# drtconway/zotmer

Measured on AMD Instinct MI355X. Metric: Gk-mers/sec kmerize k=25 on synthetic 150bp FASTQ; achieved HBM GB/s fraction, higher is better.
Workload: dtype u64

## Files before the change

### include/zotk.h

```cpp
#ifndef ZOTK_H
#define ZOTK_H

#include <stdint.h>

#ifdef __cplusplus
extern "C" {
#endif

#define ZK_OK 0
#define ZK_EINVAL (-1)
#define ZK_ENOMEM (-2)
#define ZK_EHIP (-3)
#define ZK_ENOSPC (-4)
#define ZK_EOVERFLOW (-5)
#define ZK_EINTERNAL (-6)
#define ZK_ERANGE (-7)

typedef struct zk_ctx zk_ctx;

zk_ctx* zk_create(int device, uint64_t workspace_bytes);
void zk_destroy(zk_ctx* ctx);
const char* zk_last_error(zk_ctx* ctx);
int zk_set_stream(zk_ctx* ctx, void* hip_stream);
void* zk_get_stream(zk_ctx* ctx);
int zk_sync(zk_ctx* ctx);
int zk_reserve(zk_ctx* ctx, uint64_t workspace_bytes);
int zk_release_workspace(zk_ctx* ctx);
int zk_mem_info(zk_ctx* ctx, uint64_t* free_bytes, uint64_t* total_bytes);
int zk_alloc(zk_ctx* ctx, uint64_t bytes, void** d_ptr);
int zk_free(zk_ctx* ctx, void* d_ptr);
int zk_upload(zk_ctx* ctx, void* d_dst, const void* src, uint64_t bytes);
int zk_download(zk_ctx* ctx, void* dst, const void* d_src, uint64_t bytes);
int zk_copy(zk_ctx* ctx, void* d_dst, const void* d_src, uint64_t bytes);
int zk_host_alloc(zk_ctx* ctx, uint64_t bytes, void** ptr);
int zk_host_free(zk_ctx* ctx, void* ptr);
int zk_upload_async(zk_ctx* ctx, void* d_dst, const void* src, uint64_t bytes);

#define ZK_TUNE_SORT_VARIANT 1
#define ZK_TUNE_PAIRS_VARIANT 2
#define ZK_TUNE_SHORT_SORT 3
#define ZK_TUNE_XCD_GROUP 5
#define ZK_TUNE_SIDE_DIV 4
#define ZK_TUNE_EARLY_COLLAPSE 7
#define ZK_TUNE_PACKED_PAIRS 8
#define ZK_TUNE_WIDE_TILES 9
#define ZK_TUNE_STREAM_PASS 10
#define ZK_TUNE_STREAM_RANGES 11
#define ZK_TUNE_TAG_WORDS 12
#define ZK_TUNE_DEDUPE_VARIANT 13
#define ZK_TUNE_DEDUPE_LIMIT 14
#define ZK_TUNE_DEDUPE_BITS 15
#define ZK_TUNE_COMM_CHUNK 6
#define ZK_TUNE_TAG_PASS 17
#define ZK_TUNE_KWAY 18
#define ZK_TUNE_TILE_SORT 19
#define ZK_TUNE_STRAND_BLOCKS 20
#define ZK_TUNE_COMM_SELF_LOOP 16
int zk_tune(zk_ctx* ctx, int what, int value);

#define ZK_PROF_HIST_STREAM 1
#define ZK_PROF_HIST_ARRAY 2
#define ZK_PROF_PASS_STREAM 3
#define ZK_PROF_PASS_KEYS 4
#define ZK_PROF_PASS_PAIRS 5
#define ZK_PROF_RLE 6
#define ZK_PROF_UNION 7
#define ZK_PROF_SELECT 8
#define ZK_PROF_MIRROR 9
#define ZK_PROF_INTERSECT 10
#define ZK_PROF_COUNT_HIST 11
#define ZK_PROF_PASS_PACKED 12
#define ZK_PROF_SAMPLE 13
#define ZK_PROF_TILE_SORT 14
#define ZK_PROF_CAPTURE_HITS 15
#define ZK_PROF_PROJECT_SUM 16
#define ZK_PROF_SPECTRUM 17
#define ZK_PROF_STRAND_KEYS 18
#define ZK_PROF_STRAND_PAIRS 19
#define ZK_PROF_FORMAT_PAIRS 20
#define ZK_PROF_PROBE_SCAN 21
#define ZK_PROF_BAIT_TALLY 22
#define ZK_PROF_VARS_SCAN 23
#define ZK_PROF_LINKS 24
#define ZK_PROF_LINKS_RC 25
#define ZK_PROF_CONTIG_RENDER 26
#define ZK_PROF_PILEUP 27
#define ZK_PROF_PILEUP_CUT 28
#define ZK_PROF_PULLDOWN_TALLY 29
#define ZK_PROF_CAPTURE_KMERS 30
#define ZK_PROF_PATH_SCAN 31
#define ZK_PROF_LCP_RESOLVE 32
#define ZK_PROF_SCAN_PLACE 33
#define ZK_PROF_SEQ_TALLY 34
#define ZK_PROF_SPIKE_PAIRS 35
#define ZK_PROF_SPIKE_SIZE 36
#define ZK_PROF_KSNP_FLANK 37
#define ZK_PROF_KSNP_PAIRS 38
int zk_debug_buffer(zk_ctx* ctx, void* d_buf);
int zk_profile(zk_ctx* ctx, int enable);
int zk_profile_read(zk_ctx* ctx, int tag, uint64_t* launches, double* total_ms, uint64_t* algorithmic_bytes);


int zk_pack_reads(zk_ctx* ctx, const uint8_t* d_bases, const uint64_t* d_offs, uint64_t n_reads, uint8_t* d_stream);

int zk_encode(zk_ctx* ctx, const uint8_t* d_stream, uint64_t n_bytes, int K, int both,
              uint64_t* d_out, uint64_t cap, uint64_t* n_out, uint64_t acgt[4]);

int zk_subsample(zk_ctx* ctx, const uint64_t* d_kmers, uint64_t n, uint64_t seed, double p,
                 uint64_t* d_out, uint64_t cap, uint64_t* n_out);
// ... 203 lines not shown


int zk_trim(zk_ctx* ctx, const uint64_t* d_kmers, const void* d_counts, int count_bits, uint64_t n,
            uint64_t lo, uint64_t hi, uint64_t* d_ok, void* d_oc, uint64_t cap, uint64_t* n_out);


int zk_codec64_encode(const uint64_t* vals, uint64_t n, int delta, uint64_t* words, uint64_t cap, uint64_t* n_words);
int zk_codec64_count(const uint64_t* words, uint64_t nw, uint64_t* n_values);
int zk_codec64_decode(const uint64_t* words, uint64_t nw, int delta, uint64_t* out, uint64_t cap, uint64_t* n_out);

int zk_codec64_encode_dev(zk_ctx* ctx, const uint64_t* d_vals, uint64_t n, int delta, uint64_t* d_words, uint64_t cap, uint64_t* n_words);
int zk_codec64_decode_dev(zk_ctx* ctx, const uint64_t* d_words, uint64_t nw, int delta, uint64_t* d_out, uint64_t cap, uint64_t* n_out);
int zk_codec64_encode_u32_dev(zk_ctx* ctx, const uint32_t* d_vals, uint64_t n, uint64_t* d_words, uint64_t cap, uint64_t* n_words);

int zk_undelta(zk_ctx* ctx, uint64_t* d_vals, uint64_t n, uint64_t base);
int zk_add_u64(zk_ctx* ctx, uint64_t* d_vals, uint64_t n, uint64_t x);

int zk_parse_fastq(const char* buf, uint64_t len, int final, uint64_t state[4], uint8_t* out, uint64_t out_cap,
                   uint64_t* out_len, uint64_t* consumed);
int zk_parse_fasta(const char* buf, uint64_t len, int final, uint64_t state[4], uint8_t* out, uint64_t out_cap,
                   uint64_t* out_len, uint64_t* consumed);

int zk_fastq_mask(zk_ctx* ctx, const uint8_t* d_text, uint64_t n, uint32_t line_phase, uint8_t* d_stream, uint64_t* n_newlines);

typedef struct zk_source zk_source;
zk_source* zk_source_open(zk_ctx* ctx, const char* path, int threads);
int zk_source_is_gzip(zk_source* src);
int zk_source_start(zk_source* src, uint8_t* d_dst, uint64_t cap);
int zk_source_finish(zk_source* src, uint64_t* n_bytes, int* eof);
void zk_source_close(zk_source* src);
int zk_last_newline(zk_ctx* ctx, const uint8_t* d_text, uint64_t n, uint64_t* cut);
int zk_device_to_file(zk_ctx* ctx, const void* d_src, uint64_t bytes, int fd, uint64_t file_offset, int threads);
int zk_file_to_device(zk_ctx* ctx, int fd, uint64_t file_offset, uint64_t bytes, void* d_dst, int threads);


int zk_synth_reads(zk_ctx* ctx, uint64_t seed, uint64_t first, uint64_t count, int L, uint64_t genome,
                   uint32_t sub_thr, uint32_t n_thr, uint8_t* d_stream);

int zk_checksum(zk_ctx* ctx, const uint64_t* d_kmers, const uint32_t* d_counts, uint64_t n, uint64_t sums[3]);

int zk_first_descent(zk_ctx* ctx, const uint64_t* d_kmers, uint64_t n, uint64_t* first_bad);

int zk_checksum_counts(zk_ctx* ctx, const uint64_t* d_kmers, const void* d_counts, int count_bits, uint64_t n, uint64_t sums[3]);

int zk_synth_keys(zk_ctx* ctx, uint64_t seed, uint64_t first, uint64_t count, int key_bits, uint64_t mul, uint64_t add, uint64_t mod,
                  uint64_t* d_out);
int zk_synth_counts(zk_ctx* ctx, uint64_t seed, const uint64_t* d_keys, uint64_t n, uint64_t* d_counts);

int zk_stream_checksum(zk_ctx* ctx, const uint8_t* d_stream, uint64_t n_bytes, int K, uint64_t sums[7]);

#define ZK_KEYS_FORWARD 0
#define ZK_KEYS_BOTH 1
#define ZK_KEYS_CANONICAL 2

#ifdef __cplusplus
}
#endif
#endif
```

### zotmer_amd/csrc/context.hip

```cpp
#include <stdarg.h>
#include <string.h>

#include "internal.hpp"
#include <vector>

namespace zk {

int fail(zk_ctx* c, int code, const char* fmt, ...) {
    char buf[512];
    va_list ap;
    va_start(ap, fmt);
    vsnprintf(buf, sizeof buf, fmt, ap);
    va_end(ap);
    if (c) c->last_error = buf;
    return code;
}

void arena_reset(zk_ctx* c) { c->arena_off = 0; }

int arena_alloc(zk_ctx* c, uint64_t bytes, void** p) {
    const uint64_t need = (bytes + 255) & ~255ull;
    if (c->arena_off + need > c->arena_size) {
        if (c->arena_off != 0)
            return fail(c, ZK_ENOMEM, "workspace too small: %llu bytes in use, %llu more needed, %llu reserved (call zk_reserve)",
// ... 250 lines not shown
    enter(c);
    if (workspace_bytes <= c->arena_size) return ZK_OK;
    arena_reset(c);
    void* p;
    ZK_TRY(arena_alloc(c, workspace_bytes, &p));
    arena_reset(c);
    return ZK_OK;
}

int zk_release_workspace(zk_ctx* c) {
    if (!c) return ZK_EINVAL;
    enter(c);
    ZK_HIP(c, hipStreamSynchronize(c->stream));
    if (c->arena) { ZK_HIP(c, hipFree(c->arena)); c->arena = nullptr; c->arena_size = 0; c->arena_off = 0; }
    if (c->aux) { ZK_HIP(c, hipFree(c->aux)); c->aux = nullptr; c->aux_size = 0; }
    if (c->status) { ZK_HIP(c, hipFree(c->status)); c->status = nullptr; c->status_words = 0; c->epoch = 0; }
    if (c->part16) { ZK_HIP(c, hipFree(c->part16)); c->part16 = nullptr; c->part16_words = 0; }
    return ZK_OK;
}

int zk_mem_info(zk_ctx* c, uint64_t* free_bytes, uint64_t* total_bytes) {
    if (!c) return ZK_EINVAL;
    enter(c);
    size_t f = 0, t = 0;
    ZK_HIP(c, hipMemGetInfo(&f, &t));
    if (free_bytes) *free_bytes = f;
    if (total_bytes) *total_bytes = t;
    return ZK_OK;
}

int zk_tune(zk_ctx* c, int what, int value) {
    if (!c) return ZK_EINVAL;
    enter(c);
    if (what == ZK_TUNE_SORT_VARIANT) { c->sort_variant = value; return ZK_OK; }
    if (what == ZK_TUNE_PAIRS_VARIANT) { c->pairs_variant = value; return ZK_OK; }
    if (what == ZK_TUNE_SHORT_SORT) { c->short_sort = value; return ZK_OK; }
    if (what == ZK_TUNE_SIDE_DIV) { c->side_div = value; return ZK_OK; }
    if (what == ZK_TUNE_WIDE_TILES) { c->wide_tiles = value ? 1 : 0; return ZK_OK; }
    if (what == ZK_TUNE_PACKED_PAIRS) { c->packed_pairs = value ? 1 : 0; return ZK_OK; }
    if (what == ZK_TUNE_EARLY_COLLAPSE) { c->early_collapse = value < 0 ? 0 : (value > 3 ? 3 : value); return ZK_OK; }
    if (what == ZK_TUNE_COMM_SELF_LOOP) { c->comm_self_loop = value ? 1 : 0; return ZK_OK; }
    if (what == ZK_TUNE_COMM_CHUNK) { c->comm_chunk_bytes = value > 0 ? (uint64_t)value : 0; return ZK_OK; }
    if (what == ZK_TUNE_STREAM_PASS) {
#ifdef ZK_PHASES
        c->stream_pass = value < 0 ? 0 : value;
#else
        if (value < 0 || value > 3) return fail(c, ZK_EINVAL, "stream pass variant %d (0, 1, 2 or 3)", value);
        c->stream_pass = value;
#endif
        return ZK_OK;
    }
    if (what == ZK_TUNE_TAG_WORDS) { c->tag_words = value < 0 ? 0 : (value > 2 ? 2 : value); return ZK_OK; }
    if (what == ZK_TUNE_DEDUPE_VARIANT) { c->dedupe_variant = value < 0 ? -1 : (value & 3); return ZK_OK; }
    if (what == ZK_TUNE_KWAY) { c->kway = value < 0 ? 0 : (value > 2 ? 2 : value); return ZK_OK; }
    if (what == ZK_TUNE_TILE_SORT) { c->tile_sort = value ? 1 : 0; return ZK_OK; }
    if (what == ZK_TUNE_TAG_PASS) { c->tag_pass = value ? 1 : 0; return ZK_OK; }
    if (what == ZK_TUNE_DEDUPE_BITS) { c->dedupe_bits = value < 0 ? 0 : value; return ZK_OK; }
    if (what == ZK_TUNE_STRAND_BLOCKS) { c->strand_blocks = value < 0 ? 0 : (value > 5 ? 1 : value); return ZK_OK; }
    if (what == ZK_TUNE_DEDUPE_LIMIT) { c->dedupe_limit = value < 1 ? 1 : (value > 65536 ? 65536 : value); return ZK_OK; }
    if (what == ZK_TUNE_STREAM_RANGES) { c->stream_ranges = value < 0 ? 0 : (value > 4096 ? 4096 : value); return ZK_OK; }
    if (what == ZK_TUNE_XCD_GROUP) {
        if (value < 0 || value > 32 || (value & (value - 1))) return fail(c, ZK_EINVAL, "xcd group must be 0 or a power of two <= 32");
        c->xcd_group = value;
        return ZK_OK;
    }
    return fail(c, ZK_EINVAL, "unknown tuning knob %d", what);
}

int zk_debug_buffer(zk_ctx* c, void* d_buf) {
    if (!c) return ZK_EINVAL;
    enter(c);
    c->dbg = (u64*)d_buf;
    return ZK_OK;
}

int zk_profile(zk_ctx* c, int enable) {
    if (!c) return ZK_EINVAL;
    enter(c);
    ZK_HIP(c, hipStreamSynchronize(c->stream));
    for (auto& r : c->prof) { (void)hipEventDestroy(r.a); (void)hipEventDestroy(r.b); }
    c->prof.clear();
    c->profile = enable != 0;
    return ZK_OK;
}

int zk_profile_read(zk_ctx* c, int tag, uint64_t* launches, double* total_ms, uint64_t* total_bytes) {
    if (!c) return ZK_EINVAL;
    enter(c);
    ZK_HIP(c, hipStreamSynchronize(c->stream));
    uint64_t n = 0, bytes = 0;
    double ms = 0;
    for (auto& r : c->prof) {
        if (r.tag != tag) continue;
        float t = 0;
        ZK_HIP(c, hipEventElapsedTime(&t, r.a, r.b));
        n++; ms += t; bytes += r.bytes;
    }
    if (launches) *launches = n;
    if (total_ms) *total_ms = ms;
    if (total_bytes) *total_bytes = bytes;
    return ZK_OK;
}

int zk_alloc(zk_ctx* c, uint64_t bytes, void** dptr) {
    if (!c || !dptr) return ZK_EINVAL;
    enter(c);
// ... 66 lines not shown
```

### zotmer_amd/csrc/dedupe.hpp

```cpp
#pragma once
#include "internal.hpp"

namespace zk {

struct DedupeArgs {
    const u64* kin;
    const u32* tin;
    u64 n;
    const u64* cuts;
    u64* out;
    u64* nwords;
    int tag_bits;
    int pack;
    u32* flags;
    u32* counter;
    u64* big;
    u32* n_big;
    u32 big_cap;
    u32 chunks;
    u32* sub;
    u32* bad;
    u32* n_bad;
    u32 bad_cap;
    const u32* list;
    u32* retry;
    u32* n_retry;
    u32 limit;
    u64* dbg;
    u64* m_out;
    u64* m_cursor;
    u64 m_cap;
    u64* m_hist;
    int m_K, m_passes, m_shift[2], m_bits[2];
};

#ifdef ZK_PHASES
#define DD_PHASE(k) do { if (a.dbg) { const u32 now__ = (u32)__builtin_amdgcn_s_memtime(); ph[k] += now__ - tlast; tlast = now__; } } while (0)
#else
#define DD_PHASE(k) do { } while (0)
#endif

int launch_dedupe2(zk_ctx* c, const DedupeArgs& a, bool tagin, int variant, bool unsorted);

}
```

### zotmer_amd/csrc/dedupe2.hip

```cpp
#include "dedupe.hpp"
#include <type_traits>

namespace zk {

template <int BLOCK_, int BATCH_, int ITEMS_>
struct Dedupe2Smem {
    static constexpr int BLOCK = BLOCK_, BATCH = BATCH_, ITEMS = ITEMS_, TILE = BLOCK * ITEMS, NW = BLOCK / 64, ALL = 11264, SPT = ALL / BLOCK,
                         NB = 1024, SIDE = 64 + 64 * BATCH;
    static_assert(ALL % BLOCK == 0 && ALL % 8 == 0 && ITEMS % BATCH == 0 && ITEMS % 4 == 0, "whole rounds, whole quads, whole batches");
    alignas(16) u32 keys[ALL];
    alignas(16) u32 cnt[ALL / 2];
    union {
        u32 side[NW][SIDE];
        struct { u32 bc[NB]; u32 bbase[NB + 1]; } g;
    };
    u32 ticket;
    u32 nout;
};
template <int BLOCK_, int BATCH_, int ITEMS_>
struct Dedupe2MirrorSmem : Dedupe2Smem<BLOCK_, BATCH_, ITEMS_> {
    u32 bins[2][MIRROR_RADIX];
    u64 mbase;
};

template <int ITEMS>
struct Dedupe2Next {
    u32 chunk;
    u64 lo;
    u32 len;
    u32 tag[ITEMS];
};

template <int BLOCK, int ITEMS, bool TAGIN>
__device__ __forceinline__ void dedupe2_load(const DedupeArgs& a, u64 lo, u32 pos, u32 rem, u32 tmask, u32 (&t)[ITEMS]) {
    constexpr u32 TILE = BLOCK * ITEMS;
    u32 tid = threadIdx.x;
    asm volatile("" : "+v"(tid));
    if constexpr (TAGIN) {
        const u32* tp = a.tin + lo + pos;
        if (rem >= TILE) {
            struct __attribute__((packed, aligned(4))) Tag4 { u32 a, b, c, d; };
            static_assert(ITEMS % 4 == 0, "whole quads");
#pragma unroll
            for (int i = 0; i < ITEMS / 4; i++) {
                const Tag4 q = *reinterpret_cast<const Tag4*>(tp + (u32)i * (4 * BLOCK) + 4 * tid);
                t[4 * i] = q.a; t[4 * i + 1] = q.b; t[4 * i + 2] = q.c; t[4 * i + 3] = q.d;
            }
        } else {
#pragma unroll
            for (int i = 0; i < ITEMS; i++) {
                const u32 g = (u32)i * BLOCK + tid;
                t[i] = g < rem ? tp[g] : 0u;
            }
        }
    } else {
        const u64* kp = a.kin + lo + pos;
#pragma unroll
        for (int i = 0; i < ITEMS; i++) {
            const u32 g = (u32)i * BLOCK + tid;
            t[i] = g < rem ? (u32)kp[g] & tmask : 0u;
        }
    }
}

template <class S, bool TAGIN, bool UNSORTED, bool MIRROR>
__device__ __forceinline__ void dedupe2_block(const DedupeArgs& a, S& sm, Dedupe2Next<S::ITEMS>& st, u32 (&ph)[8], u32& tlast) {
    constexpr int BLOCK = S::BLOCK, BATCH = S::BATCH, ITEMS = S::ITEMS, TILE = S::TILE, ALL = S::ALL, SPT = S::SPT, NB = S::NB;
    static_assert(!MIRROR || UNSORTED, "the mirror words are written beside the unsorted ones");
    constexpr u32 EMPTY = ~0u;
    constexpr u32 HS = ALL - 1;
    int tid = threadIdx.x;
    asm volatile("" : "+v"(tid));
    const int lane = tid & 63, wave = __builtin_amdgcn_readfirstlane(tid >> 6);
// ... 201 lines not shown
    __syncthreads();
    DD_PHASE(4);
    next_block(nchunk);
    const u64 hi_part = (u64)chunk << a.tag_bits;
    constexpr int E = 3;
    for (u32 i0 = (u32)tid; i0 < total; i0 += E * BLOCK) {
        u32 mine[E], cc[E], g0[E], g1[E], rank[E];
#pragma unroll
        for (int e = 0; e < E; e++) {
            const u32 i = i0 + e * BLOCK;
            mine[e] = sm.keys[i < total ? i : 0u];
            cc[e] = cnt16[i < total ? i : 0u];
        }
#pragma unroll
        for (int e = 0; e < E; e++) {
            const u32 b = (mine[e] >> bsh) & (NB - 1);
            g0[e] = sm.g.bbase[b]; g1[e] = sm.g.bbase[b + 1];
        }
        u32 o[E][4];
#pragma unroll
        for (int e = 0; e < E; e++)
#pragma unroll
            for (int r = 0; r < 4; r++) o[e][r] = sm.keys[g0[e] + r < (u32)ALL ? g0[e] + r : (u32)ALL - 1];
#pragma unroll
        for (int e = 0; e < E; e++) {
            rank[e] = 0;
#pragma unroll
            for (int r = 0; r < 4; r++) rank[e] += (g0[e] + r < g1[e] && o[e][r] < mine[e]) ? 1u : 0u;
            for (u32 q = g0[e] + 4; q < g1[e]; q += 4) {
                u32 p4[4];
#pragma unroll
                for (int r = 0; r < 4; r++) p4[r] = sm.keys[q + r < (u32)ALL ? q + r : (u32)ALL - 1];
#pragma unroll
                for (int r = 0; r < 4; r++) rank[e] += (q + r < g1[e] && p4[r] < mine[e]) ? 1u : 0u;
            }
        }
#pragma unroll
        for (int e = 0; e < E; e++) {
            const u32 i = i0 + e * BLOCK;
            if (i >= total) break;
            const u32 c = cc[e];
            const u64 k = hi_part | (u64)mine[e];
            if (c > maxc) {
                const u32 at = atomicAdd(a.n_big, 1u);
                if (at < a.big_cap) { a.big[2 * (u64)at] = k; a.big[2 * (u64)at + 1] = c; }
                atomicOr(a.flags, 2u);
            }
            a.out[lo + g0[e] + rank[e]] = (k << a.pack) | (u64)(c > maxc ? 0u : c);
        }
    }
    DD_PHASE(5);
}

template <int BLOCK, int BATCH, int ITEMS, bool TAGIN, bool UNSORTED, bool MIRROR = false>
__global__ __launch_bounds__(BLOCK, 2 * BLOCK / 256) void dedupe2_kernel(DedupeArgs a) {
    using S = typename std::conditional<MIRROR, Dedupe2MirrorSmem<BLOCK, BATCH, ITEMS>, Dedupe2Smem<BLOCK, BATCH, ITEMS>>::type;
    __shared__ S sm;
    static_assert(sizeof(S) <= 80 * 1024, "two workgroups per CU");
    Dedupe2Next<ITEMS> st;
    if constexpr (MIRROR)
        for (int q = threadIdx.x; q < 2 * MIRROR_RADIX; q += BLOCK) (&sm.bins[0][0])[q] = 0;
    if (threadIdx.x == 0) sm.ticket = atomicAdd(a.counter, 1u);
    __syncthreads();
    st.chunk = (u32)__builtin_amdgcn_readfirstlane((int)sm.ticket);
    st.lo = 0; st.len = 0;
    const u32 tmask = a.tag_bits >= 32 ? ~0u : (1u << a.tag_bits) - 1u;
    if (st.chunk < a.chunks) {
        const u64 nlo = a.cuts[st.chunk], nhi = a.cuts[st.chunk + 1];
        st.lo = nlo;
        st.len = nhi - nlo < (u64)a.limit ? (u32)(nhi - nlo) : ~0u;
    }
    if (st.len - 1u < ~0u - 1u) dedupe2_load<BLOCK, ITEMS, TAGIN>(a, st.lo, 0, st.len, tmask, st.tag);
    __syncthreads();
    u32 ph[8] = {0, 0, 0, 0, 0, 0, 0, 0};
    u32 tlast = a.dbg ? (u32)__builtin_amdgcn_s_memtime() : 0u;
    (void)tlast;
    u32 nblk = 0;
    while (st.chunk < a.chunks) {
        dedupe2_block<S, TAGIN, UNSORTED, MIRROR>(a, sm, st, ph, tlast);
        __syncthreads();
        DD_PHASE(6);
        nblk++;
    }
    if constexpr (MIRROR) {
        for (int q = threadIdx.x; q < a.m_passes * MIRROR_RADIX; q += BLOCK) {
            const u32 x = (&sm.bins[0][0])[q];
            if (x) atomicAdd(&a.m_hist[q], (u64)x);
        }
    }
    if (a.dbg && threadIdx.x == 0 && blockIdx.x < 256) {
        for (int k = 0; k < 8; k++) a.dbg[(u64)blockIdx.x * 16 + k] = ph[k];
        a.dbg[(u64)blockIdx.x * 16 + 8] = nblk;
    }
}

int launch_dedupe2(zk_ctx* c, const DedupeArgs& a, bool tagin, int variant, bool unsorted) {
    const u32 want = 2u * (u32)c->num_cus;
    const u32 grid = a.chunks < want ? a.chunks : want;
    if (a.m_out) {
        if (!tagin || !unsorted || !a.m_cursor || !a.m_hist || a.m_passes < 1 || a.m_passes > 2 || a.m_bits[0] > MIRROR_RBITS || a.m_bits[1] > MIRROR_RBITS)
            return fail(c, ZK_EINTERNAL, "launch_dedupe2: mirror words with %d passes, tags %d, unsorted %d", a.m_passes, (int)tagin, (int)unsorted);
        if ((variant & 3) == 1) hipLaunchKernelGGL((dedupe2_kernel<512, 1, 8, true, true, true>), dim3(grid), dim3(512), 0, c->stream, a);
        else hipLaunchKernelGGL((dedupe2_kernel<512, 2, 8, true, true, true>), dim3(grid), dim3(512), 0, c->stream, a);
        ZK_HIP(c, hipGetLastError());
        return ZK_OK;
    }
#define ZK_DD2(N, T, U) hipLaunchKernelGGL((dedupe2_kernel<512, N, 8, T, U>), dim3(grid), dim3(512), 0, c->stream, a)
#define ZK_DD2B(T, U) switch (variant & 3) { case 1: ZK_DD2(1, T, U); break; case 2: ZK_DD2(2, T, U); break; default: ZK_DD2(4, T, U); break; }
    if (unsorted) {
        if (tagin) ZK_DD2B(true, true) else ZK_DD2B(false, true)
    } else {
        if (tagin) ZK_DD2B(true, false) else ZK_DD2B(false, false)
    }
#undef ZK_DD2B
#undef ZK_DD2
    ZK_HIP(c, hipGetLastError());
    return ZK_OK;
}

}
```

### zotmer_amd/csrc/dedupe_blocks.hip

```cpp
#include "internal.hpp"
#include "dedupe.hpp"

namespace zk {

template <bool TAG32>
struct DedupeSmem {
    static constexpr int BLOCK = 1024, ITEMS = 8, TILE = BLOCK * ITEMS, NW = BLOCK / 64, ALL = TAG32 ? 12288 : 6144, SPT = ALL / BLOCK, NB = 256;
    static constexpr int SIDE_KEEP = 128, SIDE = SIDE_KEEP + 64 * ITEMS;
    typedef typename std::conditional<TAG32, u32, u64>::type E;
    E keys[ALL];
    u32 cnt[ALL];
    E side[NW][SIDE];
    u32 bc[NB];
    u32 bbase[NB + 1];
    u32 bfill[NB];
    u32 ticket;
};

__global__ void dedupe_cuts_kernel(const u64* __restrict__ k, u64 n, int tag_bits, u32 blocks, u64* __restrict__ cuts) {
    const u32 v = blockIdx.x * blockDim.x + threadIdx.x;
    if (v > blocks) return;
    u64 lo = 0, hi = n;
    while (lo < hi) {
        const u64 mid = (lo + hi) >> 1;
// ... 332 lines not shown

static int dedupe_lists(zk_ctx* c, const u64* keys, uint64_t n, int key_bits, int b, int pack, u64* work, uint64_t max_chunks,
                        const u32* tags, const u64* tag_cuts, bool unsorted, bool two_per_cu, const DedupeMirror* mirror, DedupeArgs& a, DedupeResult* r) {
    uint64_t chunks = 1ull << b;
    if (max_chunks && chunks > max_chunks) chunks = max_chunks;
    u64 *cuts, *nwords, *incl, *big;
    if (tags) {
        if (!tag_cuts || key_bits - b > 32) return fail(c, ZK_EINTERNAL, "dedupe_pass: tags of %d bits", key_bits - b);
        cuts = const_cast<u64*>(tag_cuts);
    } else ZK_TRY(arena_alloc(c, sizeof(u64) * (chunks + 1), (void**)&cuts));
    ZK_TRY(arena_alloc(c, sizeof(u64) * chunks, (void**)&nwords));
    ZK_TRY(arena_alloc(c, sizeof(u64) * chunks, (void**)&incl));
    ZK_TRY(arena_alloc(c, sizeof(u64) * 2 * DEDUPE_BIG_CAP, (void**)&big));
    a.tag_bits = key_bits - b;
    if (!tags) hipLaunchKernelGGL(dedupe_cuts_kernel, dim3((u32)div_up(chunks + 1, 256)), dim3(256), 0, c->stream, keys, (u64)n, a.tag_bits, (u32)chunks, cuts);
    a.kin = keys; a.tin = tags; a.n = n; a.cuts = cuts; a.out = work; a.nwords = nwords; a.pack = pack;
    a.chunks = (u32)chunks;
    a.flags = (u32*)&c->d_scalars->dedupe_flags;
    a.counter = (u32*)&c->d_scalars->dedupe_counter;
    a.n_big = (u32*)&c->d_scalars->dedupe_n_big;
    a.big = big; a.big_cap = DEDUPE_BIG_CAP;
    ZK_TRY(arena_alloc(c, sizeof(u32) * DEDUPE_BAD_CAP, (void**)&a.bad));
    a.bad_cap = DEDUPE_BAD_CAP;
    a.n_bad = (u32*)&c->d_scalars->dedupe_n_bad;
    a.dbg = c->dbg ? c->dbg + 8192 : nullptr;
    unsorted = unsorted && two_per_cu;
    if (!max_chunks && !unsorted && a.tag_bits >= 14 && c->arena_size - c->arena_off > 64ull * chunks * (4 + 8 + 8) + (32ull << 20) + n / 16)
        ZK_TRY(arena_alloc(c, sizeof(u32) * 64 * chunks, (void**)&a.sub));
    if (mirror && mirror->out && mirror->cap && unsorted && tags && !max_chunks && c->sort_variant == 3) {
        const PassPlan plan = sort_plan_upper(c, key_bits + pack, key_bits + pack - b);
        if (plan.passes <= 2) {
            ZK_TRY(arena_alloc(c, sizeof(u64) * MAX_PASSES * MIRROR_RADIX, (void**)&a.m_hist));
            ZK_HIP(c, hipMemsetAsync(a.m_hist, 0, sizeof(u64) * MAX_PASSES * MIRROR_RADIX, c->stream));
            a.m_out = mirror->out; a.m_cap = mirror->cap; a.m_K = mirror->K; a.m_passes = plan.passes;
            a.m_cursor = &c->d_scalars->dedupe_m_cursor;
            r->mh.passes = plan.passes; r->mh.raw = a.m_hist;
            for (int p = 0; p < plan.passes; p++) { a.m_shift[p] = r->mh.shift[p] = plan.shift[p]; a.m_bits[p] = r->mh.bits[p] = plan.bits[p]; }
            r->m_words = a.m_out; r->m_cap = a.m_cap;
        }
    }
    ZK_HIP(c, hipMemsetAsync(&c->d_scalars->dedupe_flags, 0, ZK_SPAN(dedupe_flags, dedupe_m_cursor), c->stream));
    r->cuts = cuts; r->nwords = nwords; r->incl = incl; r->big = big; r->chunks = (uint32_t)chunks; r->pack = pack; r->work = work;
    r->tag_bits = a.tag_bits; r->unsorted = unsorted;
    return ZK_OK;
}

static void launch_one_per_cu(zk_ctx* c, const DedupeArgs& d) {
    const u32 grid = d.chunks < (u32)c->num_cus ? d.chunks : (u32)c->num_cus;
    if (d.tin) hipLaunchKernelGGL((dedupe_kernel<true, true>), dim3(grid), dim3(1024), 0, c->stream, d);
    else if (d.tag_bits <= 32) hipLaunchKernelGGL((dedupe_kernel<true, false>), dim3(grid), dim3(1024), 0, c->stream, d);
    else hipLaunchKernelGGL((dedupe_kernel<false, false>), dim3(grid), dim3(1024), 0, c->stream, d);
}

static int dedupe_launch(zk_ctx* c, DedupeArgs& a, bool two_per_cu, bool unsorted, DedupeResult* r) {
    prof_begin(c, ZK_PROF_RLE, (a.tin ? 4 : 8) * a.n);
    if (two_per_cu) {
        ZK_TRY(arena_alloc(c, sizeof(u32) * a.chunks, (void**)&a.retry));
        a.n_retry = (u32*)&c->d_scalars->dedupe_n_retry;
        a.limit = (u32)c->dedupe_limit;
        ZK_TRY(launch_dedupe2(c, a, a.tin != nullptr, c->dedupe_variant, unsorted));
    } else launch_one_per_cu(c, a);
    prof_end(c);
    ZK_HIP(c, hipGetLastError());
    ZK_TRY(fetch_span(c, &c->h_scalars->dedupe_flags, ZK_SPAN(dedupe_flags, dedupe_m_cursor)));
    ZK_TRY(fetch(c, &c->h_scalars->dedupe_n_in, a.cuts + a.chunks));
    ZK_TRY(check_device_error(c));
    if (two_per_cu) { r->retry = a.retry; r->n_retry = (uint32_t)c->h_scalars->dedupe_n_retry; }
    if (a.m_out) {
        r->m_placed = c->h_scalars->dedupe_m_cursor;
        r->m_emitted = !((uint32_t)c->h_scalars->dedupe_flags & 4u) && r->m_placed <= a.m_cap;
    }
    if (two_per_cu && (uint32_t)c->h_scalars->dedupe_n_retry) {
        DedupeArgs d = a;
        d.list = a.retry; d.chunks = (uint32_t)c->h_scalars->dedupe_n_retry; d.retry = nullptr; d.n_retry = nullptr;
        ZK_HIP(c, hipMemsetAsync(a.counter, 0, sizeof(u32), c->stream));
        launch_one_per_cu(c, d);
        ZK_HIP(c, hipGetLastError());
        ZK_TRY(fetch_span(c, &c->h_scalars->dedupe_flags, ZK_SPAN(dedupe_flags, dedupe_m_cursor)));
        ZK_TRY(check_device_error(c));
    }
    return ZK_OK;
}

static int dedupe_bad_blocks(zk_ctx* c, const DedupeArgs& a, uint32_t n_bad, DedupeResult* r) {
    uint32_t list[DEDUPE_BAD_CAP];
    ZK_HIP(c, hipMemcpy(list, a.bad, sizeof(u32) * n_bad, hipMemcpyDeviceToHost));
    for (uint32_t i = 0; i < n_bad && !(r->flags & 1); i++) {
        u64 lohi[2];
        ZK_HIP(c, hipMemcpy(lohi, a.cuts + list[i], 2 * sizeof(u64), hipMemcpyDeviceToHost));
        const uint64_t m = lohi[1] - lohi[0];
        u64* res = nullptr;
        u64* bk = const_cast<u64*>(a.kin) + lohi[0];
        if (a.tin) {
            ZK_TRY(arena_alloc(c, 8 * m, (void**)&bk));
            ZK_TRY(expand_tags(c, a.tin, a.cuts, a.chunks, a.tag_bits, bk - lohi[0], list[i], 1));
        }
        ZK_TRY(sort_keys(c, bk, a.out + lohi[0], m, a.tag_bits, &res));
        if (res != bk) ZK_HIP(c, hipMemcpyAsync(bk, res, 8 * m, hipMemcpyDeviceToDevice, c->stream));
        uint64_t u = 0;
        bool ovf = false;
        ZK_TRY(rle(c, bk, m, a.out + lohi[0], nullptr, m, &u, a.pack, &ovf));
        if (ovf) { r->flags |= 1; break; }
        ZK_HIP(c, hipMemcpy(a.nwords + list[i], &u, sizeof(u64), hipMemcpyHostToDevice));
    }
    return ZK_OK;
}

int dedupe_pass(zk_ctx* c, const u64* keys, uint64_t n, int key_bits, int b, int pack, u64* work, uint64_t cap, DedupeResult* r,
                uint64_t* n_in, uint64_t max_chunks, const u32* tags, const u64* tag_cuts, bool unsorted, const DedupeMirror* mirror) {
    *r = DedupeResult();
    if (n_in) *n_in = n;
    if (n == 0) return ZK_OK;
    if (b < 1 || b > 24 || b >= key_bits || pack < 10 || pack > 31) return fail(c, ZK_EINTERNAL, "dedupe_pass: %d block bits of %d, pack %d", b, key_bits, pack);
    if (cap < n) return fail(c, ZK_ENOSPC, "dedupe_pass: work buffer of %llu words for %llu keys", (unsigned long long)cap, (unsigned long long)n);
    DedupeArgs a = {};
    const bool two_per_cu = key_bits - b <= 32 && c->dedupe_variant >= 0;
    ZK_TRY(dedupe_lists(c, keys, n, key_bits, b, pack, work, max_chunks, tags, tag_cuts, unsorted, two_per_cu, mirror, a, r));
    ZK_TRY(dedupe_launch(c, a, two_per_cu, r->unsorted, r));
    r->flags = (uint32_t)c->h_scalars->dedupe_flags;
    r->n_big = (uint32_t)c->h_scalars->dedupe_n_big;
    if (r->n_big > DEDUPE_BIG_CAP) r->flags |= 1;
    const uint32_t n_bad = (uint32_t)c->h_scalars->dedupe_n_bad;
    if (n_bad && n_bad <= DEDUPE_BAD_CAP && !(r->flags & 1) && !max_chunks) {
        ZK_TRY(dedupe_bad_blocks(c, a, n_bad, r));
        a.sub = nullptr;
    } else if (n_bad > DEDUPE_BAD_CAP) r->flags |= 1;
    ZK_HIP(c, hipMemcpyAsync(r->incl, r->nwords, sizeof(u64) * r->chunks, hipMemcpyDeviceToDevice, c->stream));
    ZK_TRY(scan64_inclusive(c, r->incl, r->chunks));
    ZK_TRY(fetch(c, &c->h_scalars->dedupe_n_out, r->incl + r->chunks - 1));
    ZK_TRY(stream_sync(c));
    r->n_out = c->h_scalars->dedupe_n_out;
    prof_add_bytes(c, ZK_PROF_RLE, 8 * r->n_out);
    r->sub = a.sub;
    if (n_in) *n_in = c->h_scalars->dedupe_n_in;
    return ZK_OK;
}

int dedupe_finish(zk_ctx* c, const DedupeResult& r, u64* out_k, u32* out_c, u64* out_m, int K, int gbases, u64** mirror_hist,
                  int* mirror_group_bits, bool packed_out) {
    if (mirror_hist) *mirror_hist = nullptr;
    int gbits = 2 * gbases;
    if (mirror_group_bits) *mirror_group_bits = gbits;
    if (r.n_out == 0) return ZK_OK;
    u64 *minc = nullptr, *place24 = nullptr;
    if (out_m && (1ull << (2 * gbases)) != r.chunks) return fail(c, ZK_EINTERNAL, "dedupe_finish: %u blocks are not 4^%d", r.chunks, gbases);
    if (out_m && r.sub && mirror_group_bits && 2 * K - gbits - 6 >= 8) {
        const uint64_t runs = 64ull * r.chunks;
        u64* minc24;
        ZK_TRY(arena_alloc(c, sizeof(u64) * runs, (void**)&minc24));
        ZK_TRY(arena_alloc(c, sizeof(u64) * runs, (void**)&place24));
        hipLaunchKernelGGL(dedupe_mirror_sizes24_kernel, dim3((u32)div_up(runs, 256)), dim3(256), 0, c->stream, r.sub, r.chunks, gbases, minc24);
        ZK_TRY(scan64_inclusive(c, minc24, runs));
        hipLaunchKernelGGL(dedupe_mirror_place24_kernel, dim3((u32)div_up(runs, 256)), dim3(256), 0, c->stream, r.sub, minc24, r.chunks, gbases, place24);
        ZK_HIP(c, hipGetLastError());
        gbits += 6;
        *mirror_group_bits = gbits;
    }
    MirrorHist mh = {};
    if (out_m && mirror_hist && c->sort_variant == 3) {
        const PassPlan plan = make_plan(2 * K - gbits, MIRROR_RBITS, gbits + r.pack);
        if (plan.passes <= 4) {
            ZK_TRY(arena_alloc(c, sizeof(u64) * MAX_PASSES * MIRROR_RADIX, (void**)&mh.raw));
            ZK_HIP(c, hipMemsetAsync(mh.raw, 0, sizeof(u64) * MAX_PASSES * MIRROR_RADIX, c->stream));
            mh.passes = plan.passes;
            for (int p = 0; p < plan.passes; p++) { mh.shift[p] = plan.shift[p]; mh.bits[p] = plan.bits[p]; }
            *mirror_hist = mh.raw;
        }
    }
    if (out_m && !place24) {
        ZK_TRY(arena_alloc(c, sizeof(u64) * r.chunks, (void**)&minc));
        hipLaunchKernelGGL(dedupe_mirror_sizes_kernel, dim3((r.chunks + 255) / 256), dim3(256), 0, c->stream, r.nwords, r.chunks, gbases, minc);
// ... 14 lines not shown
```

### zotmer_amd/csrc/encode_tile.hpp

```cpp
#pragma once
#include "common.hpp"

namespace zk {

template <int T> struct TileImage {
    static constexpr int NCH = T / 16 + 3;
    u32 codes[NCH];
    u32 valid[NCH];
};

__device__ __forceinline__ u32 record_of_thread(u32 t, u32 cpr, u32 inv) {
    return cpr == 1u ? t : (u32)(((u64)t * inv) >> 32);
}

__device__ __forceinline__ uint4 load_chunk16(const u8* __restrict__ stream, u64 n_bytes, u64 off) {
    uint4 q = make_uint4(0, 0, 0, 0);
    if (off + 16 <= n_bytes) {
        q = *reinterpret_cast<const uint4*>(stream + off);
    } else if (off < n_bytes) {
        u32 w[4] = {0, 0, 0, 0};
        for (int b = 0; b < 16; b++) {
            u32 c = (off + b < n_bytes) ? stream[off + b] : 0u;
            w[b >> 2] |= c << (8 * (b & 3));
        }
        q = make_uint4(w[0], w[1], w[2], w[3]);
    }
    return q;
}

__device__ __forceinline__ void encode_words16(const uint4 q, u32& codes, u32& vmask);

__device__ __forceinline__ void encode_chunk16(const u8* __restrict__ stream, u64 n_bytes, u64 off,
                                               u32& codes, u32& vmask) {
    encode_words16(load_chunk16(stream, n_bytes, off), codes, vmask);
}

__device__ __forceinline__ void encode_words16(const uint4 q, u32& codes, u32& vmask) {
    const u32 w[4] = {q.x, q.y, q.z, q.w};
    u32 cc = 0, vv = 0;
#pragma unroll
    for (int i = 0; i < 4; i++) {
#pragma unroll
        for (int b = 0; b < 4; b++) {
            u32 c = (w[i] >> (8 * b)) & 0xffu;
            u32 t = (c >> 1) & 3u;
            u32 code = t ^ (t >> 1);
            u32 d = (c | 0x20u) - 0x61u;
            u32 ok = (d <= 20u) ? ((0x180045u >> d) & 1u) : 0u;
            cc = (cc << 2) | code;
            vv = (vv << 1) | ok;
        }
    }
    codes = cc;
    vmask = vv;
}

// ... 99 lines not shown
```

### zotmer_amd/csrc/internal.hpp

```cpp
#pragma once
#include <hip/hip_runtime.h>
#include <stddef.h>
#include <stdint.h>
#include <stdio.h>
#include <string>
#include <vector>

#include "../../include/zotk.h"
#include "common.hpp"

struct zk_strand_counters { u32 n_declined, fail; };
struct zk_scalars {
    u64 rle_side;
    u64 total;
    u64 acgt[4];
    u64 n_keys;
    u64 rec_info[3];
    u64 sample_n;
    u64 dedupe_flags, dedupe_n_retry, dedupe_counter, dedupe_n_big, dedupe_n_bad;
    u64 dedupe_m_cursor;
    u64 dedupe_n_in;
    u64 dedupe_n_out;
    zk_strand_counters strand;
    u64 hist_big_n;
// ... 16 lines not shown
    u64 strand_sums[2];
    u64 strand_n_pairs;
    u64 format_bytes;
    u64 compact_total;
    u64 project_heads;
    u64 project_total;
    u64 spectrum[8];
    u64 table_verdict;
    u64 vars[4];
    u64 links_bad;
    u64 render_bad;
    u64 render_bytes;
    u64 pileup_cursor;
    u64 pileup_long;
    u64 pulldown_vetoed;
    u64 capkmers_bad;
    u64 capkmers_total;
    u64 path_total;
    u64 place_bad;
    u64 place_slots;
    u64 seqtally[4];
    u64 spike_bad;
    u64 spike_total[2];
    u64 ksnp_lists[2];
    u64 ksnp_tiles;
};
#define ZK_SPAN(first, last) (offsetof(zk_scalars, last) + sizeof(zk_scalars::last) - offsetof(zk_scalars, first))
static_assert(sizeof(zk_scalars) == 88 * sizeof(u64), "zk_scalars: u64 words only, no padding");
static_assert(ZK_SPAN(rle_side, total) == 2 * sizeof(u64), "rle_prefix reads rle_side and total back as one range");
static_assert(ZK_SPAN(total, acgt) == 5 * sizeof(u64), "the merges read total and acgt back as one range");
static_assert(ZK_SPAN(acgt, n_keys) == 5 * sizeof(u64) && ZK_SPAN(acgt, sample_n) == 9 * sizeof(u64),
              "sort_stream reads acgt, n_keys, rec_info and sample_n back as one range");
static_assert(ZK_SPAN(rec_info, sample_n) == 4 * sizeof(u64), "sort_stream clears rec_info and sample_n as one range");
static_assert(offsetof(zk_scalars, dedupe_n_retry) == offsetof(zk_scalars, dedupe_flags) + 8 &&
              offsetof(zk_scalars, dedupe_counter) == offsetof(zk_scalars, dedupe_flags) + 16 &&
              offsetof(zk_scalars, dedupe_n_big) == offsetof(zk_scalars, dedupe_flags) + 24 &&
              ZK_SPAN(dedupe_flags, dedupe_m_cursor) == 6 * sizeof(u64), "dedupe_pass clears and reads its six words as one range");

struct zk_ctx {
    int device = 0;
    hipStream_t stream = nullptr;
    bool own_stream = false;
    int num_cus = 256;
    int sort_variant = 3;
    int short_sort = 0;
    int packed_pairs = 1;
    int wide_tiles = 1;
    int early_collapse = 1;
    int side_div = 8;
    int pairs_variant = 7;
    int stream_pass = 1;
    int tag_words = 2;
    int dedupe_variant = 0;
    int dedupe_limit = 65536;
    int tag_pass = 0;
    int kway = 1;
    int tile_sort = 1;
    int dedupe_bits = 0;
    int strand_blocks = 1;
    int stream_ranges = 0;

    char* arena = nullptr;
    uint64_t arena_size = 0;
    uint64_t arena_off = 0;

    char* aux = nullptr;
    uint64_t aux_size = 0;

    u64* status = nullptr;
    uint64_t status_words = 0;
    unsigned short* part16 = nullptr;
    uint64_t part16_words = 0;
    u32 epoch = 0;
    u32* d_ticket = nullptr;
    u32* d_xticket = nullptr;
    int num_xcd = 1;
    int xcd_group = 0;
    u32 ticket_base = 0;

    u32* d_err = nullptr;
    zk_scalars* d_scalars = nullptr;
    zk_scalars* h_scalars = nullptr;

    std::string last_error;
    u64* dbg = nullptr;

    void* comm = nullptr;
    int comm_world = 1, comm_rank = 0;
    uint64_t comm_chunk_bytes = 0;
    int comm_self_loop = 0;

    void* ring = nullptr;

    struct ProfRec { int tag; uint64_t bytes; hipEvent_t a, b; };
    bool profile = false;
    std::vector<ProfRec> prof;
};

namespace zk {

int fail(zk_ctx* c, int code, const char* fmt, ...);
static inline void enter(zk_ctx* c) {
    int d = -1;
    if (c && (hipGetDevice(&d) != hipSuccess || d != c->device)) (void)hipSetDevice(c->device);
}
#define ZK_HIP(c, call)                                                                         \
// ... 20 lines not shown
void prof_begin(zk_ctx* c, int tag, uint64_t algorithmic_bytes);
void prof_end(zk_ctx* c);
void prof_add_bytes(zk_ctx* c, int tag, uint64_t bytes);

int fetch_span(zk_ctx* c, void* h_first, size_t bytes, const void* from = nullptr);
template <class T> static inline int fetch(zk_ctx* c, T* h_field, const void* from = nullptr) { return fetch_span(c, h_field, sizeof(T), from); }
int stream_sync(zk_ctx* c);

static inline uint64_t div_up(uint64_t a, uint64_t b) { return (a + b - 1) / b; }
static inline u32 grid_cap(const zk_ctx* c, uint64_t blocks, int per_cu) {
    const uint64_t mx = (uint64_t)c->num_cus * per_cu;
    return (u32)(blocks < mx ? blocks : mx);
}

constexpr int MAX_PASSES = 8;
struct PassPlan {
    int passes;
    int shift[MAX_PASSES];
    int bits[MAX_PASSES];
};
static inline PassPlan make_plan(int key_bits, int rbits, int lo = 0) {
    PassPlan p;
    if (key_bits < 1) key_bits = 1;
    if (key_bits > 64) key_bits = 64;
    p.passes = (key_bits + rbits - 1) / rbits;
    int base = key_bits / p.passes, rem = key_bits % p.passes, s = lo;
    for (int i = 0; i < MAX_PASSES; i++) { p.shift[i] = 0; p.bits[i] = 0; }
    for (int i = 0; i < p.passes; i++) {
        p.bits[i] = base + (i < rem ? 1 : 0);
        p.shift[i] = s;
        s += p.bits[i];
    }
    return p;
}
int sort_keys(zk_ctx* c, u64* keys, u64* alt, uint64_t n, int key_bits, u64** result);
int sort_pairs(zk_ctx* c, u64* keys, u64* alt, u32* vals, u32* valt, uint64_t n, int key_bits, u64** rk, u32** rv);
int sort_keys_upper(zk_ctx* c, u64* keys, u64* alt, uint64_t n, int key_bits, int lo_bit, u64** result, int prof_tag = ZK_PROF_PASS_PACKED);
int sort_pairs_upper(zk_ctx* c, u64* keys, u64* alt, u32* vals, u32* valt, uint64_t n, int key_bits, int lo_bit, u64** rk, u32** rv);
int sort_pairs_mirrored(zk_ctx* c, const u64* src_k, const u32* src_v, u64* keys, u64* alt, u32* vals, u32* valt, uint64_t n, int K,
                        u64** rk, u32** rv, int lo_bit = 0);
int sort_pairs_rbits(zk_ctx* c);
struct StreamSample { int shift; uint64_t value; double max_ratio; uint64_t seen = 0, distinct = 0; bool want_distinct = false; };
struct StreamTags { bool written = false; u64* cuts = nullptr; uint32_t blocks = 0; };
struct StreamSrc { const u8* stream; uint64_t n_bytes; int K; int mode; int lo_bit; int hi_bit = 0; StreamSample* sample = nullptr;
                   StreamTags* tags = nullptr; };
int sort_stream(zk_ctx* c, const StreamSrc& src, u64* buf_a, u64* buf_b, uint64_t cap, uint64_t* n_keys,
                uint64_t acgt[4], u64** result);
int sort_rbits(zk_ctx* c);
PassPlan sort_plan_upper(zk_ctx* c, int key_bits, int lo_bit);
int sort_first_bits(zk_ctx* c, int key_bits, int lo_bit);
constexpr int MIRROR_RBITS = 9, MIRROR_RADIX = 1 << MIRROR_RBITS;
struct MirrorHist { int passes; int shift[4]; int bits[4]; u64* raw; };
int sort_keys_upper_counted(zk_ctx* c, u64* keys, u64* alt, uint64_t n, int key_bits, int lo_bit, u64* counted, u64** result);
struct DedupeMirror { u64* out = nullptr; uint64_t cap = 0; int K = 0; };
struct DedupeResult {
    uint64_t n_out = 0;
    uint32_t flags = 0;
    uint32_t n_big = 0;
    u64 *cuts = nullptr, *nwords = nullptr, *incl = nullptr, *big = nullptr, *work = nullptr;
    u32* sub = nullptr;
    uint32_t chunks = 0;
    int pack = 0;
    int tag_bits = 0;
    bool unsorted = false;
    bool m_emitted = false;
    u64* m_words = nullptr;
    uint64_t m_cap = 0, m_placed = 0;
    MirrorHist mh = {};
    u32* retry = nullptr;
    uint32_t n_retry = 0;
};
int dedupe_pass(zk_ctx* c, const u64* keys, uint64_t n, int key_bits, int b, int pack, u64* work, uint64_t cap, DedupeResult* r,
                uint64_t* n_in = nullptr, uint64_t max_chunks = 0, const u32* tags = nullptr, const u64* tag_cuts = nullptr,
                bool unsorted = false, const DedupeMirror* mirror = nullptr);
int expand_tags(zk_ctx* c, const u32* tags, const u64* cuts, uint32_t blocks, int tag_bits, u64* keys_out, uint64_t first_block = 0, uint64_t n_blocks = 0);
int dedupe_finish(zk_ctx* c, const DedupeResult& r, u64* out_k, u32* out_c, u64* out_m = nullptr, int K = 0, int gbases = 0,
                  u64** mirror_hist = nullptr, int* mirror_group_bits = nullptr, bool packed_out = false);
int dedupe_sort_blocks(zk_ctx* c, DedupeResult& r);
int strand_blocks(zk_ctx* c, const DedupeResult& r, u64* keys_buf, uint64_t buf_words, int K, u64* out_k, u32* out_c, uint64_t cap,
                  uint64_t* n_out);
int collapse_pass(zk_ctx* c, const u64* keys, uint64_t n, int shift, int bits, int pack, u64* out, uint64_t cap, uint64_t* n_out,
                  uint64_t max_tiles = 0);
struct StreamRows { u32* rows = nullptr; u64* offs = nullptr; u32 ranges = 0, radix = 0; u32* gcodes = nullptr; u16* gvalid = nullptr;
                    u32 strands = 1;
                    bool wide = false; };
int stream_hist(zk_ctx* c, const u8* stream, uint64_t n_bytes, int K, int mode, const PassPlan& plan, u64* ghist, u32 gstride,
                u64* d_acgt, u64* d_n, u64* rec_info, u64* sample, u32 sample_cap, int sample_shift, u64 sample_value, u32* sample_n,
                void* image_room, uint64_t image_room_bytes, StreamRows* out);
struct StreamPlanes { u16* dig; int shift, bits; };
int stream_pass0(zk_ctx* c, uint64_t n_bytes, int K, int mode, int shift, int bits, const u64* ghist0, const StreamRows& rows,
                 uint64_t first_nl, bool uniform, u64* kout, uint64_t n, int variant, const StreamPlanes* planes = nullptr);
int stream_pass1(zk_ctx* c, const u32* tags, const u16* dig, uint64_t n, const u64* ghist0, uint32_t radix0, int bits1, u32* tout, u64* cuts);
int tile_sort_top_bits(uint64_t n, int key_bits, int rbits);
int tile_sort(zk_ctx* c, u64* keys, u32* vals, uint64_t n, int key_bits, int top, bool* declined);
int tile_sort_count(zk_ctx* c, const u64* keys, uint64_t n, int key_bits, int top, u64* uniq, u32* counts, uint64_t cap, uint64_t* n_unique,
                    bool* declined);
int trim(zk_ctx* c, const u64* keys, const void* cnts, int cbits, uint64_t n, u64 lo, u64 hi, u64* ok, void* oc,
         uint64_t cap, uint64_t* n_out);
int project_dedupe(zk_ctx* c, const u64* keys, uint64_t n, int shift, u64* out, uint64_t cap, uint64_t* n_out);
int subsample(zk_ctx* c, const u64* keys, uint64_t n, u64 seed, double p, u64* out, uint64_t cap, uint64_t* n_out);
int sample_pairs(zk_ctx* c, const u64* keys, const u64* cnts, uint64_t n, u64 seed, double p, u64* ok, u64* oc, uint64_t cap,
                 uint64_t* n_out);
int subsample_pairs(zk_ctx* c, u64* keys, u32* cnts, uint64_t n, u64 seed, double p, uint64_t* n_out);
int encode_list(zk_ctx* c, const u8* stream, uint64_t n_bytes, int K, int both, u64* out, uint64_t cap, uint64_t* n_out,
                uint64_t acgt[4]);
int capture_filter(zk_ctx* c, const u8* stream, uint64_t n_bytes, int K, const u64* baits, uint64_t n_baits, u8* out,
                   uint64_t* n_reads, uint64_t* n_kept);
// ... 37 lines not shown
```

### zotmer_amd/csrc/pipeline.hip

```cpp
#include <string.h>

#include <vector>

#include "internal.hpp"

namespace zk {

__global__ void mirror_kernel(const u64* __restrict__ c, const u32* __restrict__ n, u64 m, int K, u64* __restrict__ r,
                              u32* __restrict__ v) {
    for (u64 i = (u64)blockIdx.x * blockDim.x + threadIdx.x; i < m; i += (u64)gridDim.x * blockDim.x) {
        r[i] = revcomp(K, c[i]);
        v[i] = n[i];
    }
}

constexpr int MIRROR_GROUP_BITS = 18;
constexpr int MIRROR_GROUP_BASES = MIRROR_GROUP_BITS / 2;

__global__ void mirror_bounds_kernel(const u64* __restrict__ c, u64 n, int K, int gbits, u64* __restrict__ start) {
    const u32 g = blockIdx.x * blockDim.x + threadIdx.x;
    if (g > (1u << gbits)) return;
    const u64 want = (u64)g << (2 * K - gbits);
    u64 lo = 0, hi = n;
    if (g == (1u << gbits)) lo = n;
// ... 192 lines not shown
        ZK_TRY(sort_pairs_mirrored(c, sorted, cnt, rk, rk2, rv, rv2, uc, K, &sk, &sv));
    }
    return union_sum(c, sorted, cnt, uc, sk, sv, uc, out_k, out_c, 32, cap, n_out, nullptr, (K & 1) != 0);
}

int mirror_expand(zk_ctx* c, const u64* ck, const u32* cc, uint64_t n, int K, u64* out_k, u32* out_c, uint64_t cap, uint64_t* n_out) {
    *n_out = 0;
    if (K < 1 || K > 32) return fail(c, ZK_EINVAL, "K must be in 1..32 (got %d)", K);
    if (n == 0) return ZK_OK;
    arena_reset(c);
    const uint64_t a8 = align256(8 * n), a4 = align256(4 * n);
    int pack = 0;
    ZK_TRY(mirror_pack(c, K, cc, n, false, 0, &pack));
    const bool words = mirror_as_words(pack, K, n);
    const uint64_t wbytes = 2 * a8 + (words ? 0 : 2 * a4);
    const uint64_t need = wbytes + (9 << 20) + n / 8 + (words && n >= (1ull << 26) ? (480ull << 20) : 0);
    ZK_TRY(arena_require(c, need, need));
    char* w;
    ZK_TRY(arena_alloc(c, wbytes, (void**)&w));
    ZK_TRY(mirror_union(c, ck, cc, n, K, (u64*)w, (u64*)(w + a8), words ? nullptr : (u32*)(w + 2 * a8), words ? nullptr : (u32*)(w + 2 * a8 + a4), out_k, out_c,
                        cap, n_out, pack));
    return check_device_error(c);
}

enum CountRoute {
    COUNT_TILES,
    COUNT_BLOCKS,
    COUNT_FUSED,
    COUNT_RUNS,
    COUNT_SORTED,
    COUNT_REPLAN
};

constexpr double REPEAT_RATIO = 0.6;
static StreamSample prefix_sample(int K, int bits) { return StreamSample{2 * K - bits, (uint64_t)(0x0D71C8E5u >> (32 - bits)), REPEAT_RATIO}; }

struct KmerizePlan {
    int K;
    bool both, canonical_only;
    int rb;
    int pack;
    int collapse_bit;
    int fused_bit;
    int dedupe_bit;
    bool tags;
    int tile_top;
    int both_top;
    bool replan_pays;
    bool look;
    int look_bits;
    bool blocks_mirror;
    bool blocks_strands;
    bool blocks_unsorted;
    CountRoute low_route() const { return fused_bit ? COUNT_FUSED : collapse_bit ? COUNT_RUNS : COUNT_SORTED; }
};

static KmerizePlan plan_kmerize(const zk_ctx* c, uint64_t n_bytes, int K, bool both, bool canonical_only) {
    KmerizePlan p = {};
    p.K = K; p.both = both; p.canonical_only = canonical_only;
    const int rb = p.rb = sort_rbits(const_cast<zk_ctx*>(c));
    p.pack = c->packed_pairs ? pack_bits_for(K) : 0;
    const int lg = ilog2_ceil(n_bytes);
    if (!both && c->early_collapse) {
        const int b = rb * ((lg + 3 + rb - 1) / rb);
        if (b + rb / 2 < 2 * K) p.collapse_bit = b;
        if (p.collapse_bit >= 2 * rb && (c->early_collapse == 1 || c->early_collapse == 3) && p.pack) p.fused_bit = p.collapse_bit - rb;
    }
    if (p.fused_bit && c->early_collapse == 1) {
        const int passes = lg > 15 ? (lg - 15 + rb - 1) / rb : 1;
        const int b = rb * passes;
        if (b < p.fused_bit + rb && b + rb / 2 < 2 * K && b <= 24 && (n_bytes >> b) >= 2048) p.dedupe_bit = b;
    }
    if (!both && c->early_collapse == 1 && c->dedupe_bits > 0 && p.pack && c->dedupe_bits % rb == 0 && c->dedupe_bits + rb / 2 < 2 * K &&
        c->dedupe_bits <= 24)
        p.dedupe_bit = c->dedupe_bits;
    p.tags = p.dedupe_bit && c->tag_words && 2 * K - p.dedupe_bit <= 32;
    p.tile_top = c->tile_sort ? tile_sort_top_bits(n_bytes, 2 * K, rb) : 0;
    p.both_top = tile_sort_top_bits(2 * n_bytes, 2 * K, rb);
    p.replan_pays = !canonical_only && c->tile_sort && p.both_top;
    p.look_bits = lg - 15 < 2 ? 2 : (lg - 15 > 30 ? 30 : lg - 15);
    p.look = !p.dedupe_bit && !both && c->early_collapse && !pack_bits_for(K) && p.tile_top && p.look_bits < 2 * K;
    p.blocks_mirror = !canonical_only && p.pack && p.dedupe_bit == MIRROR_GROUP_BITS && mirror_groups(K);
    p.blocks_strands = p.blocks_mirror && (K & 1) && c->strand_blocks;
    p.blocks_unsorted = p.blocks_mirror && (K & 1) && (c->strand_blocks == 1 || c->strand_blocks >= 3);
    return p;
}

struct SortBufs {
    u64 *a, *b;
    uint64_t cap_keys;
    u64* other(const void* p) const { return p == a ? b : a; }
};
struct Output { u64* k; u32* c; uint64_t cap; uint64_t* n_out; };

struct Sorted {
    u64* keys = nullptr;
    u64* other = nullptr;
    uint64_t n = 0;
    StreamTags tags;
    bool presampled = false;
    CountRoute route = COUNT_SORTED;
};

static int sort_by_plan(zk_ctx* c, const KmerizePlan& p, const u8* stream, uint64_t n_bytes, const SortBufs& b, bool may_replan,
                        uint64_t acgt[4], Sorted* s) {
    const int K = p.K;
    StreamSrc src{stream, n_bytes, K, p.both ? ZK_KEYS_BOTH : ZK_KEYS_CANONICAL, 0};
    s->route = p.dedupe_bit ? COUNT_BLOCKS : p.low_route();
    bool sorted = false;
    if (p.dedupe_bit) {
        StreamSample smp = prefix_sample(K, p.dedupe_bit - 2);
        src.lo_bit = 2 * K - p.dedupe_bit; src.sample = &smp;
        if (p.tags) src.tags = &s->tags;
        const int rc = sort_stream(c, src, b.a, b.b, b.cap_keys, &s->n, acgt, &s->keys);
        if (rc < 0) return rc;
        src.sample = nullptr; src.tags = nullptr;
        if (rc == 1 && may_replan && p.replan_pays) { s->route = COUNT_REPLAN; return ZK_OK; }
        if (rc == 1) s->route = p.tile_top ? COUNT_TILES : p.low_route();
        else sorted = true;
        s->presampled = smp.seen >= 4096;
    } else if (p.look) {
        StreamSample smp = prefix_sample(K, p.look_bits);
        smp.want_distinct = true;
        src.lo_bit = 2 * K - p.tile_top; src.sample = &smp;
        const int rc = sort_stream(c, src, b.a, b.b, b.cap_keys, &s->n, acgt, &s->keys);
        if (rc < 0) return rc;
        src.sample = nullptr;
        if (rc != 1) { s->route = COUNT_TILES; sorted = true; }
    }
    if (!sorted) {
        if (s->route == COUNT_TILES) { src.lo_bit = 2 * K - p.tile_top; src.hi_bit = 0; }
        else { src.lo_bit = 0; src.hi_bit = p.fused_bit ? p.fused_bit : p.collapse_bit; }
        ZK_TRY(sort_stream(c, src, b.a, b.b, b.cap_keys, &s->n, acgt, &s->keys));
    }
    s->other = b.other(s->keys);
    return ZK_OK;
}

enum ListPlace {
    IN_SORT_BUF,
    IN_AUX,
    IN_OUTPUT,
    EMITTED
};
struct Counted {
    u64* keys = nullptr;
    u32* cnt = nullptr;
    uint64_t uc = 0;
    ListPlace where = IN_SORT_BUF;
    bool have_max = false;
    uint64_t max_count = 0;
    u64 *mwords = nullptr, *malt = nullptr;
    u64* mhist = nullptr;
    int mgroup = MIRROR_GROUP_BITS;
};

static int aux_list(zk_ctx* c, uint64_t m, u64** k, u32** v) {
    char* aux;
    ZK_TRY(aux_require(c, align256(8 * m) + align256(4 * m), &aux));
    *k = (u64*)aux; *v = (u32*)(aux + align256(8 * m));
    return ZK_OK;
}

static int count_sorted(zk_ctx* c, const KmerizePlan& p, const SortBufs& b, u64* keys, uint64_t n, const Output& o, Counted* r) {
    if (p.canonical_only) {
        r->where = IN_OUTPUT;
        return rle(c, keys, n, o.k, o.c, o.cap, &r->uc);
    }
    r->keys = keys; r->cnt = (u32*)b.other(keys); r->where = IN_SORT_BUF;
    return rle(c, keys, n, keys, r->cnt, n, &r->uc);
}

constexpr int ALL_BITS = -1;
static int count_by_passes(zk_ctx* c, const KmerizePlan& p, const SortBufs& b, u64* keys, uint64_t n, int lo_bit, const Output& o, Counted* r) {
    u64* res = nullptr;
    if (lo_bit == ALL_BITS) ZK_TRY(sort_keys(c, keys, b.other(keys), n, 2 * p.K, &res));
    else ZK_TRY(sort_keys_upper(c, keys, b.other(keys), n, 2 * p.K, lo_bit, &res, ZK_PROF_PASS_KEYS));
    return count_sorted(c, p, b, res, n, o, r);
}

static int reduce_words(zk_ctx* c, const KmerizePlan& p, u64* words, u64* alt, uint64_t u1, int lo_bit, Counted* r) {
    u64* res = nullptr;
    ZK_TRY(sort_keys_upper(c, words, alt, u1, 2 * p.K + p.pack, lo_bit + p.pack, &res));
    ZK_TRY(aux_list(c, u1, &r->keys, &r->cnt));
    ZK_TRY(reduce_by_key(c, res, nullptr, u1, r->keys, r->cnt, u1, &r->uc, p.pack, &r->max_count));
    r->where = IN_AUX; r->have_max = true;
    return ZK_OK;
}

static int count_tiles(zk_ctx* c, const KmerizePlan& p, const SortBufs& b, const Sorted& s, const Output& o, Counted* r) {
    bool declined = false;
    if (p.canonical_only) ZK_TRY(tile_sort_count(c, s.keys, s.n, 2 * p.K, p.tile_top, o.k, o.c, o.cap, &r->uc, &declined));
    else ZK_TRY(tile_sort_count(c, s.keys, s.n, 2 * p.K, p.tile_top, s.keys, (u32*)s.other, s.n, &r->uc, &declined));
    if (declined) return count_by_passes(c, p, b, s.keys, s.n, 0, o, r);
    r->keys = s.keys; r->cnt = (u32*)s.other; r->where = p.canonical_only ? IN_OUTPUT : IN_SORT_BUF;
    return ZK_OK;
}

static int count_blocks(zk_ctx* c, const KmerizePlan& p, const SortBufs& b, const Sorted& s, const Output& o, zk_kmerize_stats* st, Counted* r) {
    const int K = p.K, pk = p.pack;
    DedupeResult d;
    uint64_t n_in = 0;
    const uint64_t nblocks = 1ull << p.dedupe_bit, per = s.n / nblocks + 1;
    const u32* tg = s.tags.written ? (const u32*)s.keys : nullptr;
    if (!s.presampled) ZK_TRY(dedupe_pass(c, s.keys, s.n, 2 * K, p.dedupe_bit, pk, s.other, b.cap_keys, &d, &n_in, (1u << 20) / per + 4, tg, s.tags.cuts));
    if (s.presampled || (!(d.flags & 1) && (double)d.n_out <= REPEAT_RATIO * (double)n_in)) {
        DedupeMirror mo;
        const uint64_t tag_words = align256(4 * s.n) / 8;
        if (tg && p.blocks_strands && p.blocks_unsorted && c->strand_blocks != 4 && tag_words < b.cap_keys) {
            mo.out = s.keys + tag_words; mo.cap = b.cap_keys - tag_words; mo.K = K;
            if (c->strand_blocks == 5 && mo.cap > 1024) mo.cap = 1024;
        }
        ZK_TRY(dedupe_pass(c, s.keys, s.n, 2 * K, p.dedupe_bit, pk, s.other, b.cap_keys, &d, nullptr, 0, tg, s.tags.cuts, p.blocks_unsorted, &mo));
        if (!(d.flags & 1)) {
            const uint64_t uc = r->uc = d.n_out;
            const bool want_m = !(d.flags & 2) && p.blocks_mirror;
            if (want_m && p.blocks_strands && 2 * align256(8 * uc) <= 8 * b.cap_keys) {
                st->n_canonical = uc;
                r->where = EMITTED;
                return strand_blocks(c, d, s.keys, b.cap_keys, K, o.k, o.c, o.cap, o.n_out);
            }
            if (d.unsorted) ZK_TRY(dedupe_sort_blocks(c, d));
            ZK_TRY(aux_list(c, uc, &r->keys, &r->cnt));
            ZK_TRY(dedupe_finish(c, d, r->keys, r->cnt, want_m ? s.keys : nullptr, K, MIRROR_GROUP_BASES, &r->mhist, &r->mgroup, want_m));
            if (want_m) { r->mwords = s.keys; r->malt = s.other; }
            r->where = IN_AUX;
            if (!(d.flags & 2)) { r->max_count = (1ull << pk) - 1; r->have_max = true; }
            return ZK_OK;
        }
    }
    u64* keys = s.keys;
    if (tg) {
        ZK_TRY(expand_tags(c, tg, s.tags.cuts, s.tags.blocks, 2 * K - p.dedupe_bit, s.other));
        keys = s.other;
    }
    return count_by_passes(c, p, b, keys, s.n, ALL_BITS, o, r);
}

static int count_fused(zk_ctx* c, const KmerizePlan& p, const SortBufs& b, const Sorted& s, const Output& o, Counted* r) {
    const int pk = p.pack;
    const int cb = sort_first_bits(c, 2 * p.K + pk, p.fused_bit + pk);
    const uint64_t sample_tiles = 64, tile_keys = 8192;
    uint64_t us = 0, u1 = 0;
    ZK_TRY(collapse_pass(c, s.keys, s.n, p.fused_bit, cb, pk, s.other, b.cap_keys, &us, sample_tiles));
    const uint64_t m = s.n < sample_tiles * tile_keys ? s.n : sample_tiles * tile_keys;
    if ((double)us > REPEAT_RATIO * (double)m) return count_by_passes(c, p, b, s.keys, s.n, p.fused_bit, o, r);
    ZK_TRY(collapse_pass(c, s.keys, s.n, p.fused_bit, cb, pk, s.other, b.cap_keys, &u1));
    return reduce_words(c, p, s.other, s.keys, u1, p.fused_bit, r);
}

static int count_runs(zk_ctx* c, const KmerizePlan& p, const SortBufs& b, const Sorted& s, const Output& o, Counted* r) {
    const int K = p.K;
    uint64_t m = 0, heads = 0;
    ZK_TRY(sample_heads(c, s.keys, s.n, &m, &heads));
    if ((double)heads > REPEAT_RATIO * (double)m) return count_by_passes(c, p, b, s.keys, s.n, p.collapse_bit, o, r);
    if (p.pack) {
        uint64_t u1 = 0;
        bool ovf = false;
        const int rc1 = rle(c, s.keys, s.n, s.other, nullptr, b.cap_keys, &u1, p.pack, &ovf);
        if (rc1 != ZK_OK && rc1 != ZK_ENOSPC) return rc1;
// ... 296 lines not shown
```

### zotmer_amd/csrc/radix_sort.hip

```cpp
#include <stdlib.h>
#include "internal.hpp"
#include "encode_tile.hpp"

namespace zk {

constexpr int MAX_RADIX = 1024;

enum { SRC_ARRAY = 0, SRC_STREAM = 1 };

template <int BLOCK_, int ITEMS_, int RBITS_, int ROUNDS_ = 1, int WPE_ = 1, int SEG_ = 32, bool PIPE_ = false>
struct Cfg {
    static constexpr int BLOCK = BLOCK_, ITEMS = ITEMS_, RBITS = RBITS_, ROUNDS = ROUNDS_, WPE = WPE_, SEG = SEG_;
    static constexpr bool PIPE = PIPE_;
    static_assert(SEG == 0 || (BLOCK * ITEMS < 32768 && (SEG & (SEG - 1)) == 0), "16-bit tile counts");
    static constexpr int TILE = BLOCK * ITEMS, RADIX = 1 << RBITS, NW = BLOCK / 64;
    static constexpr int EXCH = TILE / ROUNDS, IPR = ITEMS / ROUNDS;
    static_assert(ITEMS % ROUNDS == 0, "ROUNDS");
    static constexpr int DPT = (RADIX + BLOCK - 1) / BLOCK;
    static_assert(ITEMS % 2 == 0 && 2 * ITEMS < 256, "ITEMS");
    static_assert(64 * ITEMS < 65536, "per-wave ranks are 16-bit");
    static_assert(RADIX <= MAX_RADIX && RBITS * MAX_PASSES >= 64, "RBITS");
};

struct SortArgs {
// ... 39 lines not shown

template <class C, int SRC, bool PAIRS, bool COUNT>
__device__ __forceinline__ u32 load_tile(const SortArgs& a, u32 tile, TileImage<C::TILE>* img, u64 (&key)[C::ITEMS],
                                         u32 (&val)[C::ITEMS], u32& acgt) {
    constexpr int TILE = C::TILE, ITEMS = C::ITEMS, BLOCK = C::BLOCK;
    const int lane = threadIdx.x & 63, wave = __builtin_amdgcn_readfirstlane((int)(threadIdx.x >> 6));
    u32 live = 0;
    if (SRC == SRC_ARRAY) {
        const u64 base = (u64)tile * TILE + (u64)wave * (64 * ITEMS) + lane;
#pragma unroll
        for (int i = 0; i < ITEMS; i++) {
            const u64 idx = base + (u64)i * 64;
            const bool ok = idx < a.n;
            key[i] = ok ? a.kin[idx] : 0ull;
            if (PAIRS) val[i] = ok ? a.vin[idx] : 0u;
            live |= (ok ? 1u : 0u) << i;
        }
        if (a.mirror_K > 0) {
#pragma unroll
            for (int i = 0; i < ITEMS; i++) key[i] = revcomp(a.mirror_K, key[i]);
        }
    } else {
        const bool both = (a.mode == ZK_KEYS_BOTH);
        const int pos_per_tile = both ? TILE / 2 : TILE;
        const u64 t0 = (u64)tile * pos_per_tile;
        for (int c = threadIdx.x; c < pos_per_tile / 16 + 3; c += BLOCK) {
            u32 cc, vv;
            encode_chunk16(a.stream, a.n_bytes, t0 + 16ull * c, cc, vv);
            img->codes[c] = cc;
            img->valid[c] = vv;
        }
        __syncthreads();
        const int K = a.K;
        if (both) {
            constexpr int H = ITEMS / 2;
#pragma unroll
            for (int i = 0; i < H; i++) {
                const int p = wave * (64 * H) + i * 64 + lane;
                u64 x;
                const bool ok = window_at(*img, p, K, x);
                const u64 xb = revcomp(K, x);
                key[i] = x;
                key[i + H] = xb;
                live |= (ok ? 1u : 0u) << i;
                live |= (ok ? 1u : 0u) << (i + H);
                if (COUNT && ok) acgt += (1u << (8 * (u32)(x & 3))) + (1u << (8 * (u32)(xb & 3)));
            }
        } else if (ITEMS == 16) {
            u64 xs[16], xr[16];
            const u32 ok16 = windows16(*img, (int)threadIdx.x, K, xs, xr);
#pragma unroll
            for (int i = 0; i < ITEMS; i++) {
                const u64 x = xs[i & 15], xb = xr[i & 15];
                key[i] = (a.mode == ZK_KEYS_CANONICAL) ? (x < xb ? x : xb) : x;
                if (COUNT && ((ok16 >> i) & 1u)) acgt += (1u << (8 * (u32)(x & 3))) + (1u << (8 * (u32)(xb & 3)));
            }
            live = ok16;
        } else {
#pragma unroll
            for (int i = 0; i < ITEMS; i++) {
                const int p = wave * (64 * ITEMS) + i * 64 + lane;
                u64 x;
                const bool ok = window_at(*img, p, K, x);
                const u64 xb = revcomp(K, x);
                key[i] = (a.mode == ZK_KEYS_CANONICAL) ? (x < xb ? x : xb) : x;
                live |= (ok ? 1u : 0u) << i;
                if (COUNT && ok) acgt += (1u << (8 * (u32)(x & 3))) + (1u << (8 * (u32)(xb & 3)));
            }
        }
    }
    return live;
}

struct HistArgs {
    SortArgs src;
    PassPlan plan;
    u64* ghist;
    u64* acgt;
    u32 tiles;
    u64* rec_info;
    u64* sample;
    u32* sample_n;
    u32 sample_cap;
    int sample_shift;
    u64 sample_value;
};

__global__ void first_newline_kernel(const u8* __restrict__ stream, u64 n_bytes, u64* out) {
    __shared__ u32 best;
    if (threadIdx.x == 0) best = 0xffffffffu;
    __syncthreads();
    const u64 lim = n_bytes < 65536 ? n_bytes : 65536;
    for (u64 i = threadIdx.x; i < lim; i += blockDim.x)
        if (stream[i] == '\n') atomicMin(&best, (u32)i);
    __syncthreads();
    if (threadIdx.x == 0) out[0] = (best == 0xffffffffu) ? ~0ull : (u64)best;
}

template <class C, int SRC> struct NextTile;
template <class C> struct NextTile<C, SRC_ARRAY> {
    u64 key[C::ITEMS];
    u32 val[C::ITEMS];
    u32 live = 0;
    template <bool PAIRS = false>
    __device__ __forceinline__ void issue(const SortArgs& a, u32 t, int tid, int wave, int lane) {
        const u64 base = (u64)t * C::TILE + (u64)wave * (64 * C::ITEMS) + lane;
        if ((u64)(t + 1) * C::TILE <= a.n) {
            const u64* p = a.kin + base;
#pragma unroll
            for (int i = 0; i < C::ITEMS; i++) key[i] = p[i * 64];
            if constexpr (PAIRS) {
                const u32* q = a.vin + base;
#pragma unroll
                for (int i = 0; i < C::ITEMS; i++) val[i] = q[i * 64];
            }
            live = (C::ITEMS >= 32) ? ~0u : ((1u << C::ITEMS) - 1u);
            return;
        }
// ... 31 lines not shown
    NextTile<C, SRC_STREAM> nx;
    nx.q0 = nx.q1 = make_uint4(0, 0, 0, 0);
    if (pre && blockIdx.x < h.tiles) nx.issue(h.src, blockIdx.x, threadIdx.x, 0, 0);
    u32 rec = 0, m = 0, step_m = 0, nl_count = 0, bad_count = 0;
    if (PRE && h.rec_info) {
        const u64 first_nl = h.rec_info[0];
        if (first_nl < 0x7fffffffull) {
            rec = (u32)first_nl + 1u;
            m = (u32)(((u64)blockIdx.x * C::TILE + 16ull * threadIdx.x) % rec);
            step_m = (u32)(((u64)gridDim.x * C::TILE) % rec);
        }
    }
    for (u32 tile = blockIdx.x; tile < h.tiles; tile += gridDim.x) {
        u64 key[C::ITEMS];
        u32 val[C::ITEMS];
        u32 pk = 0;
        u32 live = 0;
        if (pre) {
            if constexpr (PREFETCH) {
                if (rec) {
                    const u32 w4[4] = {nx.q0.x, nx.q0.y, nx.q0.z, nx.q0.w};
                    const int sep = (int)(rec - 1u) - (int)m;
                    const u64 off = (u64)tile * C::TILE + 16ull * threadIdx.x;
                    const bool expect = sep >= 0 && sep < 16 && off + (u64)sep < h.src.n_bytes;
                    bool bad = false;
#pragma unroll
                    for (int q = 0; q < 4; q++) {
                        const u32 x = w4[q] ^ 0x0a0a0a0au;
                        const u32 t = ~(((x & 0x7f7f7f7fu) + 0x7f7f7f7fu) | x | 0x7f7f7f7fu);
                        nl_count += (u32)__popc(t);
                        const u32 want = (expect && (sep >> 2) == q) ? (0x80u << (8 * (sep & 3))) : 0u;
                        bad |= (t != want);
                    }
                    bad_count += bad ? 1u : 0u;
                    m += step_m;
                    if (m >= rec) m -= rec;
                }
                u32 cc, vv;
                encode_words16(nx.q0, cc, vv);
                img.codes[threadIdx.x] = cc; img.valid[threadIdx.x] = vv;
                if (threadIdx.x + C::BLOCK < TileImage<C::TILE>::NCH) {
                    encode_words16(nx.q1, cc, vv);
                    img.codes[threadIdx.x + C::BLOCK] = cc; img.valid[threadIdx.x + C::BLOCK] = vv;
                }
                __syncthreads();
                if (tile + gridDim.x < h.tiles) nx.issue(h.src, tile + gridDim.x, threadIdx.x, 0, 0);
                Windows16<C::TILE> wg;
                wg.init(img, (int)threadIdx.x, h.src.K);
#pragma unroll
                for (int i = 0; i < 16; i++) {
                    u64 x, xb;
                    if (wg.get(i, x, xb)) {
                        pk += (1u << (8 * (u32)(x & 3))) + (1u << (8 * (u32)(xb & 3)));
                        const u64 kk = (h.src.mode == ZK_KEYS_CANONICAL) ? (x < xb ? x : xb) : x;
                        if (h.plan.passes == 2) {
                            atomicAdd(&bins[(u32)(kk >> h.plan.shift[0]) & ((1u << h.plan.bits[0]) - 1u)], 1u);
                            atomicAdd(&bins[C::RADIX + ((u32)(kk >> h.plan.shift[1]) & ((1u << h.plan.bits[1]) - 1u))], 1u);
                        } else {
#pragma unroll
                            for (int p = 0; p < MAX_PASSES; p++) {
                                if (p < h.plan.passes) {
                                    const u32 d = (u32)(kk >> h.plan.shift[p]) & ((1u << h.plan.bits[p]) - 1u);
                                    atomicAdd(&bins[p * C::RADIX + d], 1u);
                                }
                            }
                        }
                        if (h.sample && (kk >> h.sample_shift) == h.sample_value) {
                            const u32 at = atomicAdd(h.sample_n, 1u);
                            if (at < h.sample_cap) h.sample[at] = kk;
                        }
                    }
                }
                live = 0;
            }
        } else {
            if constexpr (!PRE) live = load_tile<C, SRC, false, SRC == SRC_STREAM>(h.src, tile, &img, key, val, pk);
        }
        a0 += pk & 0xffu; a1 += (pk >> 8) & 0xffu; a2 += (pk >> 16) & 0xffu; a3 += pk >> 24;
#pragma unroll
        for (int i = 0; i < C::ITEMS; i++) {
            const bool lv = (live >> i) & 1u;
#pragma unroll
            for (int p = 0; p < MAX_PASSES; p++) {
                if (p < h.plan.passes) {
                    const u32 d = (u32)(key[i] >> h.plan.shift[p]) & ((1u << h.plan.bits[p]) - 1u);
                    bool act = lv;
                    if (SRC == SRC_ARRAY) {
#pragma unroll
                        for (int r = 0; r < 2; r++) {
                            const u64 m = __ballot(act);
                            if (m == 0) break;
                            const int leader = __ffsll((long long)m) - 1;
                            const u32 dl = (u32)__builtin_amdgcn_readlane((int)d, leader);
                            const u64 same = __ballot(act && d == dl);
                            if (__popcll(same) < 8) break;
                            if ((int)(threadIdx.x & 63) == leader) atomicAdd(&bins[p * C::RADIX + dl], (u32)__popcll(same));
                            act = act && d != dl;
                        }
                    }
                    if (act) atomicAdd(&bins[p * C::RADIX + d], 1u);
                }
            }
        }
        if (SRC == SRC_STREAM) __syncthreads();
    }
    __syncthreads();
    for (int i = threadIdx.x; i < h.plan.passes * C::RADIX; i += C::BLOCK) {
// ... 444 lines not shown
        u64 key[ITEMS];
        u32 val[PAIRS ? ITEMS : 1];
        u32 rank2[ITEMS / 2];
        u32 live = 0;
        u32 tC = 0;
        bool vC = false;
        bool atomB = false;
        bool early = false;
        u32 tcB[DPT], dexB[DPT];
        u32 incB = 0, tsumB = 0;
        u64 rowA[DPT];
#pragma unroll
        for (int j = 0; j < DPT; j++) { tcB[j] = 0; dexB[j] = 0; rowA[j] = 0; }

        if (vB) {
            if constexpr (SRC == SRC_ARRAY) {
#pragma unroll
                for (int i = 0; i < ITEMS; i++) key[i] = nx.key[i];
                if constexpr (PAIRS) {
#pragma unroll
                    for (int i = 0; i < ITEMS; i++) val[i] = nx.val[i];
                    if (a.mirror_K > 0) {
#pragma unroll
                        for (int i = 0; i < ITEMS; i++) key[i] = revcomp(a.mirror_K, key[i]);
                    }
                }
                live = nx.live;
            } else {
                __syncthreads();
                const u32 nch = a.rec ? (a.rpt * a.rec) / 16 + 3 : (u32)TileImage<TILE>::NCH;
                u32 cc, vv;
                if ((u32)tid < nch) {
                    encode_words16(nx.q0, cc, vv);
                    sm.img.codes[tid] = cc; sm.img.valid[tid] = vv;
                }
                if ((u32)tid + BLOCK < nch) {
                    encode_words16(nx.q1, cc, vv);
                    sm.img.codes[tid + BLOCK] = cc; sm.img.valid[tid + BLOCK] = vv;
                }
                __syncthreads();
                u64 xs[16], xr[16];
                u32 p0 = 16u * tid_o, lim = 0xffffu;
                if (a.rec) {
                    const u32 r = record_of_thread((u32)tid_o, a.cpr, a.cpr_inv), j = tid_o - r * a.cpr;
                    p0 = r * a.rec + 16u * j;
                    const int left = (int)a.wpr - 16 * (int)j;
                    lim = (r < a.rpt) ? ((left >= 16) ? 0xffffu : ((1u << (left > 0 ? left : 0)) - 1u)) : 0u;
                    if (r >= a.rpt) p0 = 0;
                }
                live = windows16_at(sm.img, (int)p0, a.K, xs, xr) & lim;
#pragma unroll
                for (int i = 0; i < ITEMS; i++) {
                    const u64 x = xs[i & 15], xb = xr[i & 15];
                    key[i] = (a.mode == ZK_KEYS_CANONICAL) ? (x < xb ? x : xb) : x;
                }
                __syncthreads();
            }
            if constexpr (ATOM) atomB = !((a.straddle[tB >> 5] >> (tB & 31u)) & 1u);
            if (ATOM && atomB) {
                if (dirty) {
                    __syncthreads();
                    if (tid < RADIX) cnt32[tid] = 0;
                    __syncthreads();
                    dirty = false;
                }
                PSTAMP(tB, 1);
#pragma unroll
                for (int i = 0; i < ITEMS; i++) {
                    const bool lv = (live >> i) & 1u;
                    const u32 d = (u32)(key[i] >> a.shift) & dmask;
                    const u32 r = lv ? atomicAdd(&cnt32[d], 1u) : 0u;
                    if (i & 1) rank2[i / 2] |= r << 16; else rank2[i / 2] = r;
                }
            } else {
            if constexpr (ATOM) dirty = true;
            {
                u32 z = 0;
                asm volatile("" : "+v"(z));
                for (int q = lane; q < RADIX / 8; q += 64) reinterpret_cast<uint4*>(mycnt)[q] = make_uint4(z, z, z, z);
            }
#ifdef ZK_STAMPS
            asm volatile("s_waitcnt vmcnt(0)" ::: "memory");
#endif
            PSTAMP(tB, 1);
#pragma unroll
            for (int i = 0; i < ITEMS; i++) {
                const bool lv = (live >> i) & 1u;
                const u32 d = (u32)(key[i] >> a.shift) & dmask;
                u32 plo, phi;
                match_digit<C::RBITS>(d, __ballot(lv), plo, phi);
                const u32 below = __builtin_amdgcn_mbcnt_hi(phi, __builtin_amdgcn_mbcnt_lo(plo, 0u));
                const u32 npeer = (u32)__popc(plo) + (u32)__popc(phi);
                const u32 pre = lv ? (u32)mycnt[d] : 0u;
                if (i & 1) rank2[i / 2] |= (pre + below) << 16; else rank2[i / 2] = pre + below;
                if (lv && below == npeer - 1) mycnt[d] = (u16)(pre + npeer);
            }
            }
            PSTAMP(tB, 2);
            if constexpr (SRC == SRC_ARRAY) {
#pragma unroll
                for (int i = 0; i < ITEMS; i++) asm volatile("" : "+v"(key[i]));
            }
            if (tid == 0) {
                u32 t = tile_of(myx, pending, a.nx, a.glog);
                if (t >= tiles) t = steal_tile(a, myx, tiles);
                sm.ticket = t;
            }
// ... 172 lines not shown
    const u32 v = blockIdx.x, Rd = 1u << bits_d, Rin = 1u << bits_in;
    for (u32 d = threadIdx.x; d < Rd; d += blockDim.x) corr[d] = 0;
    __syncthreads();
    const u64 boundary = ghist_in[v];
    const u64 tv = boundary / tile;
    for (u64 i = tv * tile + threadIdx.x; i < boundary; i += blockDim.x) atomicAdd(&corr[(u32)(kin[i] >> shift) & (Rd - 1u)], 1u);
    __syncthreads();
    for (u32 d = threadIdx.x; d < Rd; d += blockDim.x) {
        u64 before;
        if (tv < tiles) before = status[tv * stride + d] & ZK_ST_VALUE_MASK;
        else before = (d + 1 < Rd ? ghist_d[d + 1] : n) - ghist_d[d];
        cuts[(u64)d * Rin + v] = ghist_d[d] + before + corr[d];
    }
    if (v == 0 && threadIdx.x == 0) cuts[(u64)Rd * Rin] = n;
}

int launch_wide_pass(zk_ctx* c, const SortArgs& a);

static int straddle_bitmap(zk_ctx* c, uint64_t n, u32 tile, const u64* starts, u32 buckets, u32 radix, const u32** bitmap) {
    const u32 tiles = (u32)div_up(n, tile);
    u32* bm;
    ZK_TRY(arena_alloc(c, sizeof(u32) * (tiles / 32 + 1), (void**)&bm));
    ZK_HIP(c, hipMemsetAsync(bm, 0, sizeof(u32) * (tiles / 32 + 1), c->stream));
    if (starts) {
        hipLaunchKernelGGL(straddle_kernel, dim3((radix + 255) / 256), dim3(256), 0, c->stream, starts, buckets, tile, bm);
        ZK_HIP(c, hipGetLastError());
    }
    *bitmap = bm;
    return ZK_OK;
}

struct RecInfo { uint64_t first_nl; bool uniform; };
static RecInfo uniform_records(const zk_ctx* c, uint64_t n_bytes) {
    const uint64_t first_nl = c->h_scalars->rec_info[0], nl = c->h_scalars->rec_info[1], bad = c->h_scalars->rec_info[2];
    return {first_nl, first_nl < 0x7fffffffull && n_bytes % (first_nl + 1) == 0 && bad == 0 && nl == n_bytes / (first_nl + 1)};
}

static void publish_tags(StreamTags* t, u64* cuts, uint64_t blocks) { t->cuts = cuts; t->blocks = (uint32_t)blocks; t->written = true; }

constexpr u32 SAMPLE_CAP = 1u << 20;
struct StreamPlan {
    int top;
    PassPlan plan;
    bool sampling;
    bool ranged;
    bool planes;
    bool tags;
    bool straddle;
};
static StreamPlan stream_plan(const zk_ctx* c, const StreamSrc& src, uint64_t cap, int rbits, bool pipe, uint64_t n) {
    StreamPlan s;
    s.top = (src.hi_bit > 0 && src.hi_bit < 2 * src.K) ? src.hi_bit : 2 * src.K;
    s.plan = make_plan(s.top - src.lo_bit, rbits, src.lo_bit);
    s.sampling = src.sample && cap >= 4ull * SAMPLE_CAP && src.mode == ZK_KEYS_CANONICAL;
    s.ranged = c->stream_pass != 0;
    const uint64_t n_pad = ((n + 63) & ~63ull) + 64;
    s.planes = s.ranged && c->tag_pass && src.tags && s.plan.passes == 2 && s.plan.shift[0] == 32 && s.plan.bits[0] == 9 && s.plan.bits[1] == 9 &&
               src.mode == ZK_KEYS_CANONICAL && 2 * src.K > 32 && n >= 4096 && 4 * n_pad + 2 * n + 64 <= 8 * cap;
    s.tags = src.tags && pipe && s.plan.passes == 2 && s.plan.shift[0] <= 32 && src.mode == ZK_KEYS_CANONICAL;
    s.straddle = c->tag_words >= 2 && pipe;
    return s;
}

struct RecordTiles { u32 rec = 0, rpt = 0, cpr = 0, wpr = 0, cpr_inv = 0; };
static bool record_tiles(uint64_t first_nl, int K, int block, int tile, int img_words, RecordTiles* t) {
    const uint64_t rec = first_nl + 1;
    const int64_t W = (int64_t)first_nl - K + 1;
    if (rec < 16 || W < 1) return false;
    const uint32_t cpr = (uint32_t)((W + 15) / 16);
    const uint32_t rpt = (block / cpr) / 16 * 16;
    if (!(rpt >= 16 && (uint64_t)rpt * rec / 16 + 3 <= (uint64_t)img_words && (double)rpt * (double)W > 1.02 * (double)tile * (double)W / (double)rec))
        return false;
    t->rec = (u32)rec; t->rpt = rpt; t->cpr = cpr; t->wpr = (u32)W;
    t->cpr_inv = (u32)(((1ull << 32) + cpr - 1) / cpr);
    return true;
}

template <class C>
struct Sorter {
    static int rbits() { return C::RBITS; }
    static u32 tiles_for(const SortArgs& a, int src) {
        if (src == SRC_ARRAY) return (u32)div_up(a.n, C::TILE);
        if (a.rec) return (u32)div_up(a.n_bytes / a.rec, a.rpt);
        const u64 pos = (a.mode == ZK_KEYS_BOTH) ? C::TILE / 2 : C::TILE;
        return (u32)div_up(a.n_bytes, pos);
    }

    static int begin_pass(zk_ctx* c, SortArgs& a, u32 tiles, u32 tickets, bool pipe, bool stamps = true) {
        const bool seg = !pipe && C::SEG > 0;
        ZK_TRY(lookback_begin(c, seg ? ((uint64_t)tiles / (C::SEG > 0 ? C::SEG : 1) + 2) * C::RADIX : (uint64_t)tiles * C::RADIX, tickets,
                              &a.epoch, &a.ticket_base));
        if (pipe || seg) ZK_TRY(part16_begin(c, (uint64_t)tiles * C::RADIX, &a.part));
        a.status = c->status;
        a.ticket = c->d_ticket;
        a.err = c->d_err;
        a.dbg = stamps ? c->dbg : nullptr;
        a.dbg2 = (stamps && c->dbg) ? c->dbg + 8ull * tiles : nullptr;
        return ZK_OK;
    }
    template <bool PAIRS>
    static int begin_pipe(zk_ctx* c, SortArgs& a, u32 tiles, u32* grid, bool stamps) {
        u32 g = (u32)c->num_cus * (sizeof(PipeSmem<C, PAIRS>) > 80 * 1024 ? 1 : 2);
        if (g > tiles) g = tiles;
        g += C::RADIX / 64;
        ZK_TRY(begin_pass(c, a, tiles, g, true, stamps));
        ZK_HIP(c, hipMemsetAsync(c->d_xticket, 0, 8 * 32 * sizeof(u32), c->stream));
        a.xticket = c->d_xticket;
        a.nx = 1u;
        a.glog = 0;
        *grid = g;
        return ZK_OK;
    }
// ... 412 lines not shown
```

### zotmer_amd/csrc/stream_pass.hip

```cpp
#include "internal.hpp"
#include "encode_tile.hpp"

#include <stdlib.h>
#include <type_traits>

namespace zk {

constexpr int P0_BLOCK = 512, P0_NW = 8, P0_TILE = P0_BLOCK * P0_NW, P0_IMG_WORDS = 320;
constexpr int PW_BLOCK = 1024, PW_NW = 8, PW_TILE = PW_BLOCK * PW_NW, PW_IMG_WORDS = 640;
constexpr int SH_BLOCK = 512, SH_NW = 16, SH_TILE = SH_BLOCK * SH_NW;

struct P0Geom { u32 block, nw, img_words; };
__host__ __device__ constexpr P0Geom p0_geom(bool wide) { return wide ? P0Geom{PW_BLOCK, PW_NW, PW_IMG_WORDS} : P0Geom{P0_BLOCK, P0_NW, P0_IMG_WORDS}; }

struct StreamTiling {
    u32 rec;
    u32 rpt, cpr, wpr;
    u32 cpr_inv;
    u32 tile_bytes;
    u32 ranges;
    u64 range_bytes;
};

__host__ __device__ inline StreamTiling make_tiling(u64 n_bytes, u64 first_nl, int K, u32 ranges, P0Geom g) {
// ... 81 lines not shown
    x = (x | (x << 4)) & 0x0F0F0F0Fu;
    x = (x | (x << 2)) & 0x33333333u;
    x = (x | (x << 1)) & 0x55555555u;
    return x;
}

struct SHistArgs {
    const u8* stream;
    u64 n_bytes;
    int K, mode;
    PassPlan plan;
    u32 binbase[MAX_PASSES];
    u32 nbins;
    u64* ghist;
    u32 gstride;
    u32* rows;
    u64* acgt;
    u64* rec_info;
    u64* sample;
    u32* sample_n;
    u32 sample_cap;
    int sample_shift;
    u64 sample_value;
    u32 revbase;
    u32 ranges, split;
    u32* gcodes;
    u16* gvalid;
    int dbg_atomics;
    P0Geom geom;
};

template <bool HI, bool TWO, int CANON_T = -1>
__global__ __launch_bounds__(SH_BLOCK, 4) void stream_hist_kernel(SHistArgs h) {
    extern __shared__ u32 bins[];
    __shared__ TileImage<SH_TILE> img;
    __shared__ u32 pshift[MAX_PASSES], pmask[MAX_PASSES], pbase[MAX_PASSES];
    const int tid = threadIdx.x;
    for (u32 i = tid; i < h.nbins; i += SH_BLOCK) bins[i] = 0;
    if (tid < MAX_PASSES) {
        pshift[tid] = (u32)h.plan.shift[tid] - (HI ? 32u : 0u);
        pmask[tid] = (1u << h.plan.bits[tid]) - 1u;
        pbase[tid] = h.binbase[tid];
    }
    const u64 first_nl = h.rec_info[0];
    const StreamTiling tl = make_tiling(h.n_bytes, first_nl, h.K, h.ranges, h.geom);
    const u32 w = blockIdx.x / h.split, sp = blockIdx.x % h.split;
    const u64 B = (u64)w * tl.range_bytes;
    const u64 E = (B + tl.range_bytes < h.n_bytes) ? B + tl.range_bytes : h.n_bytes;
    const u32 ntile = B < E ? (u32)((E - B + SH_TILE - 1) / SH_TILE) : 0u;
    const int K = h.K;
    const int np = h.plan.passes;
    const u64 mask = ~0ull >> (64 - 2 * K);
    const u32 mlo = (u32)mask, mhi = (u32)(mask >> 32);
    const bool canon = CANON_T == 1 ? true : h.mode == ZK_KEYS_CANONICAL;
    const bool both = CANON_T != 1 && h.mode == ZK_KEYS_BOTH;
    const u32 sh0 = (u32)h.plan.shift[0] - (HI ? 32u : 0u), sh1 = (u32)h.plan.shift[1] - (HI ? 32u : 0u);
    const u32 dm0 = (1u << h.plan.bits[0]) - 1u, dm1 = (1u << h.plan.bits[1]) - 1u;
    const u32 base1 = h.binbase[1];
    const u32 nb0 = (u32)h.plan.bits[0], nb1 = (u32)h.plan.bits[1];
    const u32 ssh = (u32)h.sample_shift - (HI ? 32u : 0u);
    const typename std::conditional<HI, u32, u64>::type sval = (typename std::conditional<HI, u32, u64>::type)h.sample_value;
    u32 a0 = 0, a1 = 0, a2 = 0, a3 = 0, nl_count = 0, bad_count = 0;
    u32 rec = 0, m = 0, step_m = 0;
    if (first_nl < 0x7fffffffull) {
        rec = (u32)first_nl + 1u;
        m = (u32)((B + (u64)sp * SH_TILE + 16ull * tid) % rec);
        step_m = (u32)(((u64)h.split * SH_TILE) % rec);
    }
    uint4 q0 = make_uint4(0, 0, 0, 0), q1 = q0;
    auto issue = [&](u32 j) {
        const u64 P = B + (u64)j * SH_TILE;
        q0 = load_chunk16(h.stream, h.n_bytes, P + 16ull * tid);
        if (tid < 3) q1 = load_chunk16(h.stream, h.n_bytes, P + 16ull * (tid + SH_BLOCK));
    };
    if (sp < ntile) issue(sp);
    __syncthreads();
    for (u32 j = sp; j < ntile; j += h.split) {
        const u64 off = B + (u64)j * SH_TILE + 16ull * tid;
        const bool mine = off < E;
        {
            u32 cc, vv;
            encode_swar16(q0, cc, vv);
            if (rec) {
                if (mine) {
                    const int sep = (int)(rec - 1u) - (int)m;
                    const bool expect = sep >= 0 && sep < 16 && off + (u64)sep < h.n_bytes;
                    const u32 sepbit = expect ? (0x8000u >> (sep & 15)) : 0u;
                    if ((vv | sepbit) == 0xffffu) {
                        const u32 wsel = (sep & 12) == 0 ? q0.x : (sep & 12) == 4 ? q0.y : (sep & 12) == 8 ? q0.z : q0.w;
                        const bool isnl = ((wsel >> (8 * (sep & 3))) & 0xffu) == 0x0au;
                        nl_count += (expect && isnl) ? 1u : 0u;
                        bad_count += (expect && !isnl) ? 1u : 0u;
                    } else {
                        const u32 w4[4] = {q0.x, q0.y, q0.z, q0.w};
                        bool bad = false;
#pragma unroll
                        for (int q = 0; q < 4; q++) {
                            const u32 x = w4[q] ^ 0x0a0a0a0au;
                            const u32 t = ~(((x & 0x7f7f7f7fu) + 0x7f7f7f7fu) | x | 0x7f7f7f7fu);
                            nl_count += (u32)__popc(t);
                            const u32 want = (expect && (sep >> 2) == q) ? (0x80u << (8 * (sep & 3))) : 0u;
                            bad |= (t != want);
                        }
                        bad_count += bad ? 1u : 0u;
                    }
                }
                m += step_m;
                if (m >= rec) m -= rec;
            }
            img.codes[tid] = cc; img.valid[tid] = vv;
            if (mine && h.gcodes) { h.gcodes[off >> 4] = cc; h.gvalid[off >> 4] = (u16)vv; }
            if (tid < 3) {
                encode_swar16(q1, cc, vv);
                img.codes[tid + SH_BLOCK] = cc; img.valid[tid + SH_BLOCK] = vv;
            }
        }
        __syncthreads();
        if (j + h.split < ntile) issue(j + h.split);
        const u64 a = ((u64)img.codes[tid] << 32) | img.codes[tid + 1];
        const u64 b = ((u64)img.codes[tid + 2] << 32) | img.codes[tid + 3];
        u64 v = ((u64)img.valid[tid] << 48) | ((u64)img.valid[tid + 1] << 32) | ((u64)img.valid[tid + 2] << 16) | (u64)img.valid[tid + 3];
        v = runs_of_k(v, K);
        const u32 V16 = mine ? (u32)(v >> 48) : 0u;
        WindowWords<SH_NW> ww;
        ww.init(a, b, 0u, K);
        if (h.acgt) {
            const u32 Vs = spread16(V16);
            const u32 ff = (u32)(a >> 32);
            const u32 fl = (u32)((K > 1 ? ((a << (2 * K - 2)) | (b >> (66 - 2 * K))) : a) >> 32);
            const u32 lf = ff & Vs, hf = (ff >> 1) & Vs, ll = fl & Vs, hl = (fl >> 1) & Vs;
            a0 += (u32)__popc(Vs & ~hl & ~ll) + (u32)__popc(hf & lf);
            a1 += (u32)__popc(~hl & ll) + (u32)__popc(hf & ~lf);
            a2 += (u32)__popc(hl & ~ll) + (u32)__popc(~hf & lf);
            a3 += (u32)__popc(hl & ll) + (u32)__popc(Vs & ~hf & ~lf);
        }
        u32 hits = 0;
#pragma unroll
        for (int i = 0; i < SH_NW; i++) {
            const u32 inc = (V16 >> (15 - i)) & 1u;
            typename std::conditional<HI, u32, u64>::type kd;
            if constexpr (HI) {
                const u32 xh = ww.xhi(i) & mhi, bh = ww.bhi(i) & mhi;
                kd = canon ? (xh < bh ? xh : bh) : xh;
            } else {
                const u64 x = ((u64)(ww.xhi(i) & mhi) << 32) | (ww.xlo(i) & mlo), xb = ((u64)(ww.bhi(i) & mhi) << 32) | (ww.blo(i) & mlo);
                kd = canon ? (x < xb ? x : xb) : x;
            }
            if constexpr (TWO && HI) {
#ifdef ZK_PHASES
                if (h.dbg_atomics >= 1) atomicAdd(&bins[__builtin_amdgcn_ubfe(kd, sh0, nb0)], inc);
                if (h.dbg_atomics >= 2) atomicAdd(&bins[base1 + __builtin_amdgcn_ubfe(kd, sh1, nb1)], inc);
                if (h.dbg_atomics == 0) a0 += kd & inc;
#else
                atomicAdd(&bins[__builtin_amdgcn_ubfe(kd, sh0, nb0)], inc);
                atomicAdd(&bins[base1 + __builtin_amdgcn_ubfe(kd, sh1, nb1)], inc);
#endif
            } else if constexpr (TWO) {
                atomicAdd(&bins[(u32)(kd >> sh0) & dm0], inc);
                atomicAdd(&bins[base1 + ((u32)(kd >> sh1) & dm1)], inc);
            } else {
                for (int p = 0; p < np; p++) atomicAdd(&bins[pbase[p] + ((u32)(kd >> pshift[p]) & pmask[p])], inc);
                if (both) {
                    typename std::conditional<HI, u32, u64>::type kr;
                    if constexpr (HI) kr = ww.bhi(i) & mhi;
                    else kr = ((u64)(ww.bhi(i) & mhi) << 32) | (ww.blo(i) & mlo);
                    atomicAdd(&bins[h.revbase + ((u32)(kr >> pshift[0]) & pmask[0])], inc);
                    for (int p = 1; p < np; p++) atomicAdd(&bins[pbase[p] + ((u32)(kr >> pshift[p]) & pmask[p])], inc);
                }
            }
            if constexpr (HI) {
                if (h.sample) hits |= ((kd >> ssh) == sval ? 1u : 0u) << (15 - i);
            } else if (h.sample && inc && (kd >> ssh) == sval) {
                const u32 at = atomicAdd(h.sample_n, 1u);
                if (at < h.sample_cap) h.sample[at] = kd;
            }
        }
        hits &= V16;
        if (HI && hits) {
#pragma unroll
            for (int i = 0; i < SH_NW; i++) {
                if ((hits >> (15 - i)) & 1u) {
                    const u64 x = (((u64)ww.xhi(i) << 32) | ww.xlo(i)) & mask, xb = (((u64)ww.bhi(i) << 32) | ww.blo(i)) & mask;
                    const u64 kk = canon ? (x < xb ? x : xb) : x;
                    const u32 at = atomicAdd(h.sample_n, 1u);
                    if (at < h.sample_cap) h.sample[at] = kk;
                }
            }
        }
        __syncthreads();
    }
    __syncthreads();
    const u32 r0 = 1u << h.plan.bits[0];
    for (u32 i = tid; i < h.nbins; i += SH_BLOCK) {
        const u32 c = bins[i];
        if (!c) continue;
        if (i < r0) atomicAdd(&h.rows[(u64)w * r0 + i], c);
        if (both && i >= h.revbase) {
            atomicAdd(&h.rows[(u64)(h.ranges + w) * r0 + (i - h.revbase)], c);
            atomicAdd(&h.ghist[i - h.revbase], (u64)c);
            continue;
        }
        int p = 0;
        for (int q = 1; q < np; q++) if (i >= pbase[q]) p = q;
        atomicAdd(&h.ghist[(u64)p * h.gstride + (i - pbase[p])], (u64)c);
    }
    if (rec) {
        nl_count = wave_sum_u32(nl_count); bad_count = wave_sum_u32(bad_count);
        if ((tid & 63) == 0) {
            if (nl_count) atomicAdd(&h.rec_info[1], (u64)nl_count);
            if (bad_count) atomicAdd(&h.rec_info[2], (u64)bad_count);
        }
    }
    if (h.acgt) {
        a0 = wave_sum_u32(a0); a1 = wave_sum_u32(a1); a2 = wave_sum_u32(a2); a3 = wave_sum_u32(a3);
        if ((tid & 63) == 0) {
            if (a0) atomicAdd(&h.acgt[0], (u64)a0);
            if (a1) atomicAdd(&h.acgt[1], (u64)a1);
            if (a2) atomicAdd(&h.acgt[2], (u64)a2);
            if (a3) atomicAdd(&h.acgt[3], (u64)a3);
        }
    }
}

__global__ void rows_scan_kernel(const u32* __restrict__ rows, const u64* __restrict__ ghist0, u32 ranges, u32 radix, u64* __restrict__ offs) {
    const u32 d = blockIdx.x * blockDim.x + threadIdx.x;
    if (d >= radix) return;
    u64 run = ghist0[d];
    for (u32 w = 0; w < ranges; w++) {
        offs[(u64)w * radix + d] = run;
        run += rows[(u64)w * radix + d];
    }
}

struct P0Args {
    const u32* gcodes;
    const u16* gvalid;
    u64 n_bytes;
    int K;
    StreamTiling tl;
    u32 ranges;
    int by_record;
    int shift, bits;
    const u64* offs;
    const u32* rows;
    u64* kout;
    u16* dig_out;
    int dig_shift;
    u32 dig_mask;
    u64 n;
    u32* err;
    int split_stores;
    int dbg_mode;
    u64* dbg;
};
#ifdef ZK_PHASES
#define P0_MODE (a.dbg_mode)
#define P0_PHASE(k) do { if (a.dbg) { const u32 now__ = (u32)__builtin_amdgcn_s_memtime(); ph[k] += now__ - tlast; tlast = now__; } } while (0)
#else
#define P0_MODE 0
#define P0_PHASE(k) do { } while (0)
#endif

__device__ __forceinline__ u32 wave_incl_scan_dpp(u32 v) {
    v += (u32)__builtin_amdgcn_update_dpp(0, (int)v, 0x111, 0xf, 0xf, false);
    v += (u32)__builtin_amdgcn_update_dpp(0, (int)v, 0x112, 0xf, 0xf, false);
    v += (u32)__builtin_amdgcn_update_dpp(0, (int)v, 0x114, 0xf, 0xf, false);
    v += (u32)__builtin_amdgcn_update_dpp(0, (int)v, 0x118, 0xf, 0xf, false);
    v += (u32)__builtin_amdgcn_update_dpp(0, (int)v, 0x142, 0xa, 0xf, false);
    v += (u32)__builtin_amdgcn_update_dpp(0, (int)v, 0x143, 0xc, 0xf, false);
    return v;
}

__device__ __forceinline__ u32 unit_pack(u32 slot, u32 len, u32 digit) { return slot | ((len - 1u) << 14) | (digit << 18); }

template <int RBITS, int G>
struct P0Smem {
    static constexpr int RADIX = 1 << RBITS, CAP = P0_TILE + RADIX * (G - 1), UNITS = CAP / G + 2 * RADIX;
    u64 exch[CAP + 64];
    u64 gbase[RADIX];
    u32 units[UNITS];
    u32 codes[P0_IMG_WORDS], valid[P0_IMG_WORDS];
    u32 cnt[RADIX + 64];
    u16 off[RADIX];
    u16 nu[RADIX];
    u32 nunits;
    u32 anybad;
};

template <int RBITS, int G, bool CANON, bool FAST, bool PLANES = false>
__global__ __launch_bounds__(P0_BLOCK, 4) void stream_pass0_kernel(P0Args a) {
    using S = P0Smem<RBITS, G>;
    constexpr int RADIX = S::RADIX, NW = P0_NW, BLOCK = P0_BLOCK;
    static_assert(S::CAP < (1 << 14) && G <= 16 && RBITS <= 14, "unit_pack");
    static_assert(RADIX == BLOCK && (G & (G - 1)) == 0 && 64 % G == 0, "one digit per thread; whole units per wave instruction");
    __shared__ S sm;
    const int tid = threadIdx.x, lane = tid & 63, wave = __builtin_amdgcn_readfirstlane(tid >> 6);
    const u32 w = blockIdx.x;
    const bool rev = !CANON && w >= a.ranges;
    const u32 radix = 1u << a.bits;
    const u64 B = (u64)(rev ? w - a.ranges : w) * a.tl.range_bytes;
    if (B >= a.n_bytes) return;
    const u64 E = (B + a.tl.range_bytes < a.n_bytes) ? B + a.tl.range_bytes : a.n_bytes;
    const u32 tile_bytes = a.by_record ? a.tl.tile_bytes : (u32)P0_TILE;
    const u32 ntile = (u32)((E - B + tile_bytes - 1) / tile_bytes);
    const u32 nch = tile_bytes / 16 + 3;
    const int K = a.K;
    const u64 mask = ~0ull >> (64 - 2 * K);
    const u32 mlo = (u32)mask, mhi = (u32)(mask >> 32);
    const u32 dmask = radix - 1u;
    const u32 nchunks = (u32)((a.n_bytes + 15) >> 4);
    auto digit = [&](u64 k) -> u32 {
        if constexpr (FAST) return __builtin_amdgcn_ubfe((u32)(k >> 32), (u32)a.shift - 32u, (u32)a.bits);
        else return (u32)(k >> a.shift) & dmask;
    };
    u64 F = (u32)tid < radix ? a.offs[(u64)w * radix + tid] : 0ull;
    const u64 Fend = F + ((u32)tid < radix ? a.rows[(u64)w * radix + tid] : 0u);
    u32 nck = 0, ctail = 0;
    u32 bad = 0;
    u32 flen_dbg = 0;
    sm.cnt[tid] = 0;
    if (tid == 0) sm.anybad = 0;
    u32 p0 = (u32)NW * tid, wlim = (1u << NW) - 1u;
    if (a.by_record) {
        const u32 r = record_of_thread((u32)tid, a.tl.cpr, a.tl.cpr_inv), j = tid - r * a.tl.cpr;
        p0 = r * a.tl.rec + (u32)NW * j;
        const int left = (int)a.tl.wpr - NW * (int)j;
        wlim = (r < a.tl.rpt) ? ((left >= NW) ? (1u << NW) - 1u : ((1u << (left > 0 ? left : 0)) - 1u)) : 0u;
        if (r >= a.tl.rpt) p0 = 0;
    }
    u32 qc = 0, qv = 0;
    auto fetch = [&](u64 T) {
        const u64 idx = (T >> 4) + (u32)tid;
        const bool in = (u32)tid < nch && idx < nchunks;
        qc = in ? a.gcodes[idx] : 0u;
        qv = in ? (u32)a.gvalid[idx] : 0u;
    };
    fetch(B);
    if ((u32)tid < nch) { sm.codes[tid] = qc; sm.valid[tid] = qv; }
    if (ntile > 1) fetch(B + tile_bytes);
    __syncthreads();
    u32 ph[8] = {0, 0, 0, 0, 0, 0, 0, 0};
    u32 tlast = a.dbg ? (u32)__builtin_amdgcn_s_memtime() : 0;
    (void)tlast;
// ... 87 lines not shown
            for (int g = 0; g < NF; g++) {
                const u32 sl = e4[g] & 0x3fffu;
                u32 hw[8];
#pragma unroll
                for (int q = 0; q < 8; q++) hw[q] = (u32)(sm.exch[sl + q] >> 32);
#pragma unroll
                for (int q = 0; q < 4; q++)
                    d8[g][q] = ((hw[2 * q] >> (a.dig_shift - 32)) & a.dig_mask) | (((hw[2 * q + 1] >> (a.dig_shift - 32)) & a.dig_mask) << 16);
                b4[g] = sm.gbase[(e4[g] >> 18) & (u32)(RADIX - 1)];
            }
#pragma unroll
            for (int g = 0; g < NF; g++) asm volatile("" : "+v"(d8[g][0]), "+v"(d8[g][1]), "+v"(d8[g][2]), "+v"(d8[g][3]), "+v"(b4[g]));
#pragma unroll
            for (int g = 0; g < NF; g++) {
                const u32 u = base + g * BLOCK + (u32)tid;
                const u32 len = ((e4[g] >> 14) & 15u) + 1u;
                u16* dst = a.dig_out + (b4[g] + (e4[g] & 0x3fffu));
                if (u < end && P0_MODE != 1) {
                    if (len == 8) { Dig8 v; v.a = d8[g][0]; v.b = d8[g][1]; v.c = d8[g][2]; v.d = d8[g][3]; *reinterpret_cast<Dig8*>(dst) = v; }
                    else {
#pragma unroll
                        for (int q = 0; q < 7; q++) if ((u32)q < len) dst[q] = (u16)(d8[g][q >> 1] >> (16 * (q & 1)));
                    }
                }
            }
        }
    };
    u32 held = 0, held_end = 0;
    for (u32 t = 0; t < ntile; t++) {
        const u64 T0 = B + (u64)t * tile_bytes;
        const bool last = t + 1 == ntile;
        if (P0_MODE == 2 && t > 1) {
            __syncthreads();
            sm.gbase[tid] += flen_dbg;
            __syncthreads();
        } else {
        u64 key[NW];
        u32 live;
        {
            const u32 j = p0 >> 4, s = p0 & 15u;
            const u64 sa = ((u64)sm.codes[j] << 32) | sm.codes[j + 1];
            const u64 sb = ((u64)sm.codes[j + 2] << 32) | sm.codes[j + 3];
            u64 v = ((u64)sm.valid[j] << 48) | ((u64)sm.valid[j + 1] << 32) | ((u64)sm.valid[j + 2] << 16) | (u64)sm.valid[j + 3];
            v = runs_of_k(v, K);
            live = (__brev((u32)((v << s) >> (64 - NW))) >> (32 - NW)) & wlim;
            if (T0 + p0 >= E) live = 0;
            WindowWords<NW> ww;
            ww.init(sa, sb, s, K);
#pragma unroll
            for (int i = 0; i < NW; i++) {
                const u64 x = ((u64)(ww.xhi(i) & mhi) << 32) | (FAST ? ww.xlo(i) : (ww.xlo(i) & mlo));
                if constexpr (CANON) {
                    const u64 xb = ((u64)(ww.bhi(i) & mhi) << 32) | (FAST ? ww.blo(i) : (ww.blo(i) & mlo));
                    key[i] = x < xb ? x : xb;
                } else {
                    const u64 xb = ((u64)(ww.bhi(i) & mhi) << 32) | (FAST ? ww.blo(i) : (ww.blo(i) & mlo));
                    key[i] = rev ? xb : x;
                }
            }
        }
        u64 ck[G - 1];
#pragma unroll
        for (int j = 0; j < G - 1; j++) ck[j] = sm.exch[ctail + j];
        u32 rk[NW];
#pragma unroll
        for (int i = 0; i < NW; i++) {
            rk[i] = atomicAdd(&sm.cnt[((live >> i) & 1u) ? digit(key[i]) : (u32)RADIX + (u32)lane], 1u);
        }
        if constexpr (!PLANES) { if (held < held_end) store_units(held, held_end, std::integral_constant<int, 2>()); }
        held = held_end = 0;
        P0_PHASE(0);
        __syncthreads();
        P0_PHASE(1);
        u32 O, tot, flen, head, nu;
        {
            const uint4 c0 = reinterpret_cast<const uint4*>(sm.cnt)[2 * lane], c1 = reinterpret_cast<const uint4*>(sm.cnt)[2 * lane + 1];
            const u32 s8 = c0.x + c0.y + c0.z + c0.w + c1.x + c1.y + c1.z + c1.w;
            const u32 inc8 = wave_incl_scan_dpp(s8);
            const u32 before = wave ? (u32)__builtin_amdgcn_readlane((int)inc8, 8 * wave - 1) : 0u;
            tot = sm.cnt[tid];
            const u32 inc = wave_incl_scan_dpp(tot);
            O = before + inc - tot;
            u64 end = F + tot;
            if (end > Fend) { bad = 1; sm.anybad = 1; end = Fend > F ? Fend : F; }
            u64 Eo = last ? end : (end & ~(u64)(G - 1));
            if (Eo < F) Eo = F;
            flen = (u32)(Eo - F);
            head = (u32)(F & (G - 1)) ? G - (u32)(F & (G - 1)) : 0u;
            if (head > flen) head = flen;
            nu = (head ? 1u : 0u) + (flen - head + G - 1) / G;
            sm.nu[tid] = (u16)nu;
        }
        __syncthreads();
        {
            const uint4 c0 = reinterpret_cast<const uint4*>(sm.nu)[lane];
            const u32 s2 = c0.x + c0.y + c0.z + c0.w;
            const u32 s8 = (s2 & 0xffffu) + (s2 >> 16);
            const u32 inc8 = wave_incl_scan_dpp(s8);
            const u32 before = wave ? (u32)__builtin_amdgcn_readlane((int)inc8, 8 * wave - 1) : 0u;
            const u32 inc = wave_incl_scan_dpp(nu);
            u32 U = before + inc - nu;
            if (tid == 0) sm.nunits = (u32)__builtin_amdgcn_readlane((int)inc8, 63);
            sm.off[tid] = (u16)O;
            sm.cnt[tid] = tot - flen;
            sm.gbase[tid] = F - O;
            flen_dbg = flen;
            u32 slot = O, left = flen;
// ... 18 lines not shown
            }
#pragma unroll
            for (int j = 0; j < G - 1; j++) sm.exch[((u32)j < nck && O + j < (u32)S::CAP) ? O + j : (u32)S::CAP + (u32)lane] = ck[j];
            nck = tot - flen;
            ctail = O + flen;
        }
        P0_PHASE(3);
        __syncthreads();
        P0_PHASE(4);
        if (!last) {
            if ((u32)tid < nch) { sm.codes[tid] = qc; sm.valid[tid] = qv; }
            if (t + 2 < ntile) fetch(T0 + 2ull * tile_bytes);
        }
        P0_PHASE(5);
        }
        {
            const u32 nunits = (sm.anybad || sm.nunits > (u32)S::UNITS) ? 0u : sm.nunits;
            const u32 half = (PLANES || P0_MODE == 2 || !a.split_stores) ? nunits : (nunits / 2 + 127u) & ~127u;
            if constexpr (PLANES) store_units_planes(0, half < nunits ? half : nunits);
            else store_units(0, half < nunits ? half : nunits, std::integral_constant<int, 4>());
            held = half < nunits ? half : nunits; held_end = nunits;
        }
        P0_PHASE(6);
        __syncthreads();
        P0_PHASE(7);
    }
    if constexpr (!PLANES) { if (held < held_end) store_units(held, held_end, std::integral_constant<int, 2>()); }
    if (a.dbg && tid == 0) {
        for (int k = 0; k < 8; k++) a.dbg[(u64)w * 16 + k] = (u64)ph[k];
        a.dbg[(u64)w * 16 + 8] = ntile;
    }
    if (P0_MODE) return;
    if (bad || ((u32)tid < radix && (F != Fend || nck != 0))) atomicOr(a.err, ZK_DERR_MISMATCH);
}

template <int RBITS, int G>
struct P0WideSmem {
    static constexpr int RADIX = 1 << RBITS, CARRY = G - 1;
    static constexpr int DEAD = PW_TILE, CB = PW_TILE + 64;
    static constexpr int SLOTS = CB + RADIX * CARRY;
    static constexpr int UNITS = (PW_TILE + RADIX * CARRY) / G + 2 * RADIX;
    u64 exch[SLOTS];
    u64 gbase[RADIX];
    u32 units[UNITS];
    u32 codes[PW_IMG_WORDS], valid[PW_IMG_WORDS];
    alignas(16) u32 cnt[RADIX + 64];
    u32 mv[RADIX];
    u16 off[RADIX];
    alignas(16) u16 nu[RADIX];
    u32 nunits;
    u32 anybad;
};

template <int RBITS, bool CANON, bool FAST>
__global__ __launch_bounds__(PW_BLOCK) void stream_pass0_wide_kernel(P0Args a) {
    constexpr int G = 16;
    using S = P0WideSmem<RBITS, G>;
    constexpr int RADIX = S::RADIX, NW = PW_NW, BLOCK = PW_BLOCK;
    static_assert(2 * RADIX == BLOCK, "one digit per thread of waves 0-7");
    static_assert(S::SLOTS < (1 << 14) && S::CARRY < 16 && RBITS <= 9, "unit words");
    static_assert(sizeof(S) <= 160 * 1024, "LDS of a CU");
    __shared__ S sm;
    const int tid = threadIdx.x, lane = tid & 63, wave = __builtin_amdgcn_readfirstlane(tid >> 6);
    const bool owner = wave < RADIX / 64;
    const u32 w = blockIdx.x;
    const bool rev = !CANON && w >= a.ranges;
    const u32 radix = 1u << a.bits;
    const u64 B = (u64)(rev ? w - a.ranges : w) * a.tl.range_bytes;
    if (B >= a.n_bytes) return;
    const u64 E = (B + a.tl.range_bytes < a.n_bytes) ? B + a.tl.range_bytes : a.n_bytes;
    const u32 tile_bytes = a.by_record ? a.tl.tile_bytes : (u32)PW_TILE;
    const u32 ntile = (u32)((E - B + tile_bytes - 1) / tile_bytes);
    const u32 nch = tile_bytes / 16 + 3;
    const int K = a.K;
    const u64 mask = ~0ull >> (64 - 2 * K);
    const u32 mlo = (u32)mask, mhi = (u32)(mask >> 32);
    const u32 dmask = radix - 1u;
    const u32 nchunks = (u32)((a.n_bytes + 15) >> 4);
    auto digit = [&](u64 k) -> u32 {
        if constexpr (FAST) return __builtin_amdgcn_ubfe((u32)(k >> 32), (u32)a.shift - 32u, (u32)a.bits);
        else return (u32)(k >> a.shift) & dmask;
    };
    const bool mine = owner && (u32)tid < radix;
    u64 F = mine ? a.offs[(u64)w * radix + tid] : 0ull;
    const u64 Fend = F + (mine ? a.rows[(u64)w * radix + tid] : 0u);
    u32 r = 0;
    u32 bad = 0;
    u32 flen_dbg = 0;
    if (tid < RADIX + 64) sm.cnt[tid] = 0;
    if (owner) sm.mv[tid] = 0;
    if (tid == 0) { sm.anybad = 0; sm.units[0] = 0; }
    u32 p0 = (u32)NW * tid, wlim = (1u << NW) - 1u;
    if (a.by_record) {
        const u32 rr = record_of_thread((u32)tid, a.tl.cpr, a.tl.cpr_inv), j = tid - rr * a.tl.cpr;
        p0 = rr * a.tl.rec + (u32)NW * j;
        const int left = (int)a.tl.wpr - NW * (int)j;
        wlim = (rr < a.tl.rpt) ? ((left >= NW) ? (1u << NW) - 1u : ((1u << (left > 0 ? left : 0)) - 1u)) : 0u;
        if (rr >= a.tl.rpt) p0 = 0;
    }
    u32 qc = 0, qv = 0;
    auto fetch = [&](u64 T) {
        const u64 idx = (T >> 4) + (u32)tid;
        const bool in = (u32)tid < nch && idx < nchunks;
        qc = in ? a.gcodes[idx] : 0u;
        qv = in ? (u32)a.gvalid[idx] : 0u;
    };
    fetch(B);
    if ((u32)tid < nch) { sm.codes[tid] = qc; sm.valid[tid] = qv; }
// ... 14 lines not shown
            for (int g = 0; g < NF; g++) {
                const u32 u = base + g * GROUPS + g0;
                e4[g] = sm.units[u < end ? u : 0u];
            }
#pragma unroll
            for (int g = 0; g < NF; g++) asm volatile("" : "+v"(e4[g]));
#pragma unroll
            for (int g = 0; g < NF; g++) {
                const u32 d = (e4[g] >> 18) & (u32)(RADIX - 1), kc = e4[g] >> 27;
                const u32 cs = (u32)S::CB + (u32)S::CARRY * d, ps = (e4[g] & 0x3fffu) - 16u;
                k4[g] = sm.exch[j < kc ? cs + j : ps + j];
                l4[g] = sm.exch[j + 1 < kc ? cs + j + 1 : ps + j + 1];
                b4[g] = sm.gbase[d];
            }
#pragma unroll
            for (int g = 0; g < NF; g++) asm volatile("" : "+v"(k4[g]), "+v"(l4[g]), "+v"(b4[g]));
#pragma unroll
            for (int g = 0; g < NF; g++) {
                const u32 u = base + g * GROUPS + g0;
                const u32 len1 = (e4[g] >> 14) & 15u;
                u64* dst = a.kout + (b4[g] + (e4[g] & 0x3fffu) + j);
                const bool fits = P0_MODE != 2 || b4[g] + (e4[g] & 0x3fffu) + G <= a.n;
                if (u < end && P0_MODE != 1 && fits) {
                    if (j < len1) { Key2 v; v.a = k4[g]; v.b = l4[g]; *reinterpret_cast<Key2*>(dst) = v; }
                    else if (j == len1) *dst = k4[g];
                }
            }
        }
    };
    for (u32 t = 0; t < ntile; t++) {
        const u64 T0 = B + (u64)t * tile_bytes;
        const bool last = t + 1 == ntile;
        if (P0_MODE == 2 && t > 1) {
            __syncthreads();
            if (owner) sm.gbase[tid] += flen_dbg;
            __syncthreads();
        } else {
        u64 key[NW];
        u32 live;
        {
            const u32 j = p0 >> 4, s = p0 & 15u;
            const u64 sa = ((u64)sm.codes[j] << 32) | sm.codes[j + 1];
            const u64 sb = ((u64)sm.codes[j + 2] << 32) | sm.codes[j + 3];
            u64 v = ((u64)sm.valid[j] << 48) | ((u64)sm.valid[j + 1] << 32) | ((u64)sm.valid[j + 2] << 16) | (u64)sm.valid[j + 3];
            v = runs_of_k(v, K);
            live = (__brev((u32)((v << s) >> (64 - NW))) >> (32 - NW)) & wlim;
            if (T0 + p0 >= E) live = 0;
            WindowWords<NW> ww;
            ww.init(sa, sb, s, K);
#pragma unroll
            for (int i = 0; i < NW; i++) {
                const u64 x = ((u64)(ww.xhi(i) & mhi) << 32) | (FAST ? ww.xlo(i) : (ww.xlo(i) & mlo));
                const u64 xb = ((u64)(ww.bhi(i) & mhi) << 32) | (FAST ? ww.blo(i) : (ww.blo(i) & mlo));
                if constexpr (CANON) key[i] = x < xb ? x : xb;
                else key[i] = rev ? xb : x;
            }
        }
        u32 rk[NW];
#pragma unroll
        for (int i = 0; i < NW; i++) rk[i] = atomicAdd(&sm.cnt[((live >> i) & 1u) ? digit(key[i]) : (u32)RADIX + (u32)lane], 1u);
        P0_PHASE(0);
        __syncthreads();
        P0_PHASE(1);
        u32 O = 0, tot = 0, flen = 0, head = 0, nu = 0, c = 0;
        if (owner) {
            const uint4 c0 = reinterpret_cast<const uint4*>(sm.cnt)[2 * lane], c1 = reinterpret_cast<const uint4*>(sm.cnt)[2 * lane + 1];
            const u32 s8 = c0.x + c0.y + c0.z + c0.w + c1.x + c1.y + c1.z + c1.w;
            const u32 inc8 = wave_incl_scan_dpp(s8);
            const u32 before = wave ? (u32)__builtin_amdgcn_readlane((int)inc8, 8 * wave - 1) : 0u;
            c = sm.cnt[tid];
            const u32 inc = wave_incl_scan_dpp(c);
            O = before + inc - c;
            tot = r + c;
            u64 end = F + tot;
            if (end > Fend) { bad = 1; sm.anybad = 1; end = Fend > F ? Fend : F; }
            u64 Eo = last ? end : (end & ~(u64)(G - 1));
            if (Eo < F) Eo = F;
            flen = (u32)(Eo - F);
            head = (u32)(F & (G - 1)) ? G - (u32)(F & (G - 1)) : 0u;
            if (head > flen) head = flen;
            nu = (head ? 1u : 0u) + (flen - head + G - 1) / G;
            sm.off[tid] = (u16)O;
            sm.nu[tid] = (u16)nu;
        } else {
            const u32 q = (u32)tid - (u32)RADIX, j = 2u * (q & 7u);
#pragma unroll
            for (int h = 0; h < 2; h++) {
                u32 m4[4], d4[4];
                u64 v4[4], x4[4];
#pragma unroll
                for (int g = 0; g < 4; g++) { d4[g] = (u32)(4 * h + g) * (RADIX / 8) + (q >> 3); m4[g] = sm.mv[d4[g]]; }
#pragma unroll
                for (int g = 0; g < 4; g++) asm volatile("" : "+v"(m4[g]));
#pragma unroll
                for (int g = 0; g < 4; g++) {
                    const u32 n = m4[g] >> 18, src = m4[g] & 0x3fffu;
                    v4[g] = sm.exch[j < n ? src + j : (u32)S::DEAD + (u32)lane];
                    x4[g] = sm.exch[j + 1 < n ? src + j + 1 : (u32)S::DEAD + (u32)lane];
                }
#pragma unroll
                for (int g = 0; g < 4; g++) asm volatile("" : "+v"(v4[g]), "+v"(x4[g]));
#pragma unroll
                for (int g = 0; g < 4; g++) {
                    const u32 n = m4[g] >> 18, dst = (u32)S::CB + (u32)S::CARRY * d4[g] + ((m4[g] >> 14) & 15u);
                    sm.exch[j < n ? dst + j : (u32)S::DEAD + (u32)lane] = v4[g];
                    sm.exch[j + 1 < n ? dst + j + 1 : (u32)S::DEAD + (u32)lane] = x4[g];
                }
// ... 59 lines not shown
    }
    if (a.dbg && tid == 0) {
        for (int k = 0; k < 8; k++) a.dbg[(u64)w * 16 + k] = (u64)ph[k];
        a.dbg[(u64)w * 16 + 8] = ntile;
    }
    if (P0_MODE) return;
    if (bad || (mine && (F != Fend || r != 0))) atomicOr(a.err, ZK_DERR_MISMATCH);
}

static bool p0_wide(const zk_ctx* c) { return (c->stream_pass & 0xff) == 1 && !c->tag_pass; }

int stream_ranges(zk_ctx* c, bool wide) { return c->stream_ranges > 0 ? c->stream_ranges : (wide ? 1 : 2) * (c->num_cus > 0 ? c->num_cus : 1); }

int stream_hist(zk_ctx* c, const u8* stream, uint64_t n_bytes, int K, int mode, const PassPlan& plan, u64* ghist, u32 gstride,
                u64* d_acgt, u64* d_n, u64* rec_info, u64* sample, u32 sample_cap, int sample_shift, u64 sample_value, u32* sample_n,
                void* image_room, uint64_t image_room_bytes, StreamRows* out) {
    SHistArgs h = {};
    h.stream = stream; h.n_bytes = n_bytes; h.K = K; h.mode = mode; h.plan = plan;
    u32 nb = 0;
    bool hi = 2 * K > 32;
    for (int p = 0; p < plan.passes; p++) { h.binbase[p] = nb; nb += 1u << plan.bits[p]; if (plan.shift[p] < 32) hi = false; }
    if (sample && sample_shift < 32) hi = false;
    const bool both = mode == ZK_KEYS_BOTH;
    const u32 strands = both ? 2u : 1u;
    h.revbase = nb;
    if (both) nb += 1u << plan.bits[0];
    h.nbins = nb;
    h.ghist = ghist; h.gstride = gstride;
    h.acgt = d_acgt; h.rec_info = rec_info;
    h.sample = sample; h.sample_n = sample_n; h.sample_cap = sample_cap; h.sample_shift = sample_shift; h.sample_value = sample_value;
    const bool wide = p0_wide(c);
    h.geom = p0_geom(wide);
    h.ranges = (u32)stream_ranges(c, wide);
    h.split = wide ? 8 : 4;
    h.dbg_atomics = 2;
#ifdef ZK_PHASES
    if (const char* e = getenv("ZK_HIST_ATOMICS")) h.dbg_atomics = atoi(e);
#endif
    const u32 r0 = 1u << plan.bits[0];
    const uint64_t nchunks = (n_bytes + 15) / 16;
    u32* rows; u64* offs;
    ZK_TRY(arena_alloc(c, sizeof(u32) * (uint64_t)strands * h.ranges * r0, (void**)&rows));
    ZK_TRY(arena_alloc(c, sizeof(u64) * (uint64_t)strands * h.ranges * r0, (void**)&offs));
    const uint64_t codes_bytes = (sizeof(u32) * nchunks + 255) & ~255ull, image_bytes = codes_bytes + ((sizeof(u16) * nchunks + 255) & ~255ull);
    char* img = nullptr;
    if (image_room && image_room_bytes >= image_bytes + 256) img = (char*)(((uintptr_t)image_room + image_room_bytes - image_bytes) & ~(uintptr_t)255);
    else ZK_TRY(arena_alloc(c, image_bytes, (void**)&img));
    h.gcodes = (u32*)img; h.gvalid = (u16*)(img + codes_bytes);
    h.rows = rows;
    ZK_HIP(c, hipMemsetAsync(rows, 0, sizeof(u32) * (uint64_t)strands * h.ranges * r0, c->stream));
    ZK_HIP(c, hipMemsetAsync(ghist, 0, sizeof(u64) * MAX_PASSES * gstride, c->stream));
    if (d_acgt) ZK_HIP(c, hipMemsetAsync(d_acgt, 0, sizeof(u64) * 4, c->stream));
    const u32 grid = h.ranges * h.split;
    prof_begin(c, ZK_PROF_HIST_STREAM, n_bytes);
    const bool two = plan.passes == 2 && !both;
    if (hi && two && mode == ZK_KEYS_CANONICAL) hipLaunchKernelGGL((stream_hist_kernel<true, true, 1>), dim3(grid), dim3(SH_BLOCK), nb * sizeof(u32), c->stream, h);
    else if (hi && two) hipLaunchKernelGGL((stream_hist_kernel<true, true>), dim3(grid), dim3(SH_BLOCK), nb * sizeof(u32), c->stream, h);
    else if (hi) hipLaunchKernelGGL((stream_hist_kernel<true, false>), dim3(grid), dim3(SH_BLOCK), nb * sizeof(u32), c->stream, h);
    else if (two) hipLaunchKernelGGL((stream_hist_kernel<false, true>), dim3(grid), dim3(SH_BLOCK), nb * sizeof(u32), c->stream, h);
    else hipLaunchKernelGGL((stream_hist_kernel<false, false>), dim3(grid), dim3(SH_BLOCK), nb * sizeof(u32), c->stream, h);
    prof_end(c);
    ZK_HIP(c, hipGetLastError());
    out->rows = rows; out->offs = offs; out->ranges = h.ranges; out->strands = strands; out->radix = r0; out->gcodes = h.gcodes; out->gvalid = h.gvalid;
    out->wide = wide;
    return ZK_OK;
}

int stream_pass0(zk_ctx* c, uint64_t n_bytes, int K, int mode, int shift, int bits, const u64* ghist0, const StreamRows& rows,
                 uint64_t first_nl, bool uniform, u64* kout, uint64_t n, int variant, const StreamPlanes* planes) {
    if (bits < 1 || bits > 9 || (1u << bits) != rows.radix) return fail(c, ZK_EINTERNAL, "stream_pass0: %d digit bits, rows of %u", bits, rows.radix);
    if ((mode == ZK_KEYS_BOTH) != (rows.strands == 2)) return fail(c, ZK_EINTERNAL, "stream_pass0: rows of %u strands for mode %d", rows.strands, mode);
    const u32 grid = rows.ranges * rows.strands;
    hipLaunchKernelGGL(rows_scan_kernel, dim3((rows.radix + 255) / 256), dim3(256), 0, c->stream, rows.rows, ghist0, grid, rows.radix, rows.offs);
    P0Args a = {};
    a.gcodes = rows.gcodes; a.gvalid = rows.gvalid; a.n_bytes = n_bytes; a.K = K;
    a.tl = make_tiling(n_bytes, first_nl, K, rows.ranges, p0_geom(rows.wide));
    a.ranges = rows.ranges;
    a.by_record = (uniform && a.tl.rec) ? 1 : 0;
    a.shift = shift; a.bits = bits; a.offs = rows.offs; a.rows = rows.rows; a.kout = kout; a.n = n; a.err = c->d_err; a.dbg = c->dbg; a.dbg_mode = variant >> 8; a.split_stores = (variant & 0xff) == 3;
    const bool canon = mode == ZK_KEYS_CANONICAL, fast = 2 * K > 32 && shift >= 32;
    if (planes) {
        if (!canon || !fast || rows.wide) return fail(c, ZK_EINTERNAL, "stream_pass0: planes need the canonical fast plan and the 512-thread kernel");
        a.dig_out = planes->dig; a.dig_shift = planes->shift; a.dig_mask = (1u << planes->bits) - 1u;
        prof_begin(c, ZK_PROF_PASS_STREAM, n_bytes + 6 * n);
        hipLaunchKernelGGL((stream_pass0_kernel<9, 8, true, true, true>), dim3(rows.ranges), dim3(P0_BLOCK), 0, c->stream, a);
        prof_end(c);
        ZK_HIP(c, hipGetLastError());
        return ZK_OK;
    }
    prof_begin(c, ZK_PROF_PASS_STREAM, n_bytes + 8 * n);
    if (rows.wide) {
        if (canon && fast) hipLaunchKernelGGL((stream_pass0_wide_kernel<9, true, true>), dim3(grid), dim3(PW_BLOCK), 0, c->stream, a);
        else if (canon) hipLaunchKernelGGL((stream_pass0_wide_kernel<9, true, false>), dim3(grid), dim3(PW_BLOCK), 0, c->stream, a);
        else if (fast) hipLaunchKernelGGL((stream_pass0_wide_kernel<9, false, true>), dim3(grid), dim3(PW_BLOCK), 0, c->stream, a);
        else hipLaunchKernelGGL((stream_pass0_wide_kernel<9, false, false>), dim3(grid), dim3(PW_BLOCK), 0, c->stream, a);
    } else if (canon && fast) hipLaunchKernelGGL((stream_pass0_kernel<9, 8, true, true>), dim3(grid), dim3(P0_BLOCK), 0, c->stream, a);
    else if (canon) hipLaunchKernelGGL((stream_pass0_kernel<9, 8, true, false>), dim3(grid), dim3(P0_BLOCK), 0, c->stream, a);
    else if (fast) hipLaunchKernelGGL((stream_pass0_kernel<9, 8, false, true>), dim3(grid), dim3(P0_BLOCK), 0, c->stream, a);
    else hipLaunchKernelGGL((stream_pass0_kernel<9, 8, false, false>), dim3(grid), dim3(P0_BLOCK), 0, c->stream, a);
    prof_end(c);
    ZK_HIP(c, hipGetLastError());
    return ZK_OK;
}

}
```

### zotmer_amd/native.py

```python
import ctypes as C
import os

import numpy as np

_HERE = os.path.dirname(os.path.abspath(__file__))
LIB_PATH = os.environ.get("ZOTK_LIB") or os.path.join(_HERE, "libzotk.so")

ZK_OK, ZK_EINVAL, ZK_ENOMEM, ZK_EHIP, ZK_ENOSPC, ZK_EOVERFLOW, ZK_EINTERNAL, ZK_ERANGE = 0, -1, -2, -3, -4, -5, -6, -7
KMERIZE_CANONICAL, KMERIZE_BOTH, KMERIZE_SUBSAMPLE, KMERIZE_CANONICAL_ONLY = 0, 1, 2, 4
STRAND_ORPHANS = 1
PROBE_TILE, PROBE_MAX_WINDOWS = 4096, 1024
TALLY_TILE = 2048
CONTIG_TILE = 4096
VARS_TILE = 4096
LINKS_TILE = 1024
NO_LINK = 0xFFFFFFFF
PILEUP_DIAGS, PILEUP_TILE = 256, 4096
PATH_TILE, PATH_CHUNK = 4096, 256
LCP_TILE = 256
SEQTALLY_TILE = 4096
KSNP_HAMMING, KSNP_LEVENSHTEIN = 0, 1
KSNP_WAVE_GROUP, KSNP_LDS_GROUP, KSNP_PAIR_TILE = 64, 1024, 256
DEFAULT_TAG_WORDS = 2

# ... 352 lines not shown
        class _Pinned:
            def __init__(s):
                s.ptr, s.n = p.value, int(nbytes)
                s.array = np.ctypeslib.as_array((C.c_uint8 * max(s.n, 1)).from_address(s.ptr))[:s.n]

            def free(s):
                if s.ptr and ctx.h:
                    s.array = None
                    ctx.lib.zk_host_free(ctx.h, s.ptr)
                s.ptr = None

            def __del__(s):
                try:
                    s.free()
                except Exception:
                    pass
        return _Pinned()

    def upload_async(self, dst, src_ptr, nbytes):
        self._check(self.lib.zk_upload_async(self.h, dst.ptr, src_ptr, int(nbytes)))

    IO_THREADS = int(os.environ.get("ZOT_IO_THREADS", 0)) or max(1, min(8, (os.cpu_count() or 2) - 1))

    def source_open(self, path, threads=None):
        return Source(self, path, threads or self.IO_THREADS)

    def last_newline(self, text, n):
        cut = C.c_uint64(0)
        self._check(self.lib.zk_last_newline(self.h, text.ptr, int(n), C.byref(cut)))
        return cut.value

    def device_to_file(self, arr, fileno, offset, threads=None):
        self._check(self.lib.zk_device_to_file(self.h, arr.ptr, arr.nbytes, int(fileno), int(offset), threads or self.IO_THREADS))

    def file_to_device(self, fileno, offset, nbytes, dtype=np.uint8, threads=None):
        dt = np.dtype(dtype)
        out = self.empty(nbytes // dt.itemsize, dt)
        self._check(self.lib.zk_file_to_device(self.h, int(fileno), int(offset), int(nbytes), out.ptr, threads or self.IO_THREADS))
        return out

    def upload_stream(self, data):
        a = np.frombuffer(data, dtype=np.uint8) if isinstance(data, (bytes, bytearray, memoryview)) else np.asarray(data, np.uint8)
        return self.upload(a)

    PROF_TAGS = {"hist_stream": 1, "hist_array": 2, "pass_stream": 3, "pass_keys": 4, "pass_pairs": 5, "rle": 6,
                 "union_sum": 7, "select": 8, "mirror": 9, "intersect": 10, "count_hist": 11, "pass_packed": 12, "sample": 13, "tile_sort": 14,
                 "capture_hits": 15, "project_sum": 16, "spectrum": 17, "strand_keys": 18, "strand_pairs": 19, "format_pairs": 20,
                 "probe_scan": 21, "bait_tally": 22, "vars_scan": 23, "links": 24, "links_rc": 25, "contig_render": 26,
                 "pileup": 27, "pileup_cut": 28, "pulldown_tally": 29, "capture_kmers": 30, "path_scan": 31, "lcp_resolve": 32, "scan_place": 33,
                 "seq_tally": 34, "spike_pairs": 35, "spike_size": 36, "ksnp_flank": 37, "ksnp_pairs": 38}

    TUNE_IDS = dict(sort_variant=1, pairs_variant=2, short_sort=3, side_div=4, xcd_group=5, comm_chunk=6, early_collapse=7,
                    packed_pairs=8, wide_tiles=9, stream_pass=10, stream_ranges=11, tag_words=12, dedupe_variant=13, dedupe_limit=14,
                    dedupe_bits=15, comm_self_loop=16, tag_pass=17, kway=18, tile_sort=19, strand_blocks=20)

    def tune(self, **knobs):
        for name in knobs:
            if name not in self.TUNE_IDS:
                raise TypeError("tune() got an unexpected keyword argument %r" % name)
        for name, value in knobs.items():
            if value is not None:
                self._check(self.lib.zk_tune(self.h, self.TUNE_IDS[name], int(value)))

    def profile(self, enable=True):
        self._check(self.lib.zk_profile(self.h, int(enable)))

    def profile_read(self):
        out = {}
        for name, tag in self.PROF_TAGS.items():
            n, b, ms = C.c_uint64(0), C.c_uint64(0), C.c_double(0)
            self._check(self.lib.zk_profile_read(self.h, tag, C.byref(n), C.byref(ms), C.byref(b)))
            if n.value:
                out[name] = dict(launches=n.value, ms=ms.value, bytes=b.value)
        return out

    def pack_reads(self, bases, offs):
        n_reads = offs.n - 1
        total = int(offs.to_host()[-1]) if offs.n else 0
        out = self.empty(total + n_reads, np.uint8)
        self._check(self.lib.zk_pack_reads(self.h, bases.ptr, offs.ptr, n_reads, out.ptr))
        return out

    def encode(self, stream, K, both=True):
        cap = stream.n * (2 if both else 1)
        out = self.empty(cap, np.uint64)
        n = C.c_uint64(0)
        acgt = (C.c_uint64 * 4)()
        self._check(self.lib.zk_encode(self.h, stream.ptr, stream.n, K, int(both), out.ptr, cap, C.byref(n), acgt))
        return out.view(n.value), [int(v) for v in acgt]

    def subsample(self, kmers, seed, p):
        out = self.empty(kmers.n, np.uint64)
        n = C.c_uint64(0)
        self._check(self.lib.zk_subsample(self.h, kmers.ptr, kmers.n, int(seed), float(p), out.ptr, kmers.n, C.byref(n)))
        return out.view(n.value)

    def can(self, K, kmers):
        out = self.empty(kmers.n, np.uint64)
        self._check(self.lib.zk_can(self.h, int(K), kmers.ptr, kmers.n, out.ptr))
        self.sync()
        return out

    def sort_keys(self, keys, key_bits):
        self._check(self.lib.zk_sort_keys(self.h, keys.ptr, keys.n, key_bits))
        return keys

    def sort_pairs(self, keys, vals, key_bits):
# ... 612 lines not shown
```

Before: 166.5.

## Key odd-K k-mers by middle-base strand rule and shrink dedupe table for occupancy

For odd K, adds a key mode that picks the strand by the middle base instead of comparing the forward and reverse-complement words, so the min-compare is replaced by a bit-select in the histogram and scatter passes. The mode is wired through the stream histogram, pass0 kernels and sampling, and is enabled in the plan when mirror strand blocks are in use. It also adds a smaller LDS table variant of the mirror dedupe kernel that fits three workgroups per CU, chosen when the estimated distinct keys per block fit. This raises occupancy, but the table can overflow on skewed blocks, and the per-block estimate depends on sampling.

```diff
diff --git a/include/zotk.h b/include/zotk.h
--- a/include/zotk.h
+++ b/include/zotk.h
@@ -55,6 +55,7 @@
 #define ZK_TUNE_KWAY 18
 #define ZK_TUNE_TILE_SORT 19
 #define ZK_TUNE_STRAND_BLOCKS 20
+#define ZK_TUNE_DEDUPE_TABLE 21
 #define ZK_TUNE_COMM_SELF_LOOP 16
 int zk_tune(zk_ctx* ctx, int what, int value);
 
@@ -364,6 +365,7 @@
 #define ZK_KEYS_FORWARD 0
 #define ZK_KEYS_BOTH 1
 #define ZK_KEYS_CANONICAL 2
+#define ZK_KEYS_MIDDLE 3
 
 #ifdef __cplusplus
 }
diff --git a/zotmer_amd/csrc/context.hip b/zotmer_amd/csrc/context.hip
--- a/zotmer_amd/csrc/context.hip
+++ b/zotmer_amd/csrc/context.hip
@@ -326,6 +326,7 @@
     }
     if (what == ZK_TUNE_TAG_WORDS) { c->tag_words = value < 0 ? 0 : (value > 2 ? 2 : value); return ZK_OK; }
     if (what == ZK_TUNE_DEDUPE_VARIANT) { c->dedupe_variant = value < 0 ? -1 : (value & 3); return ZK_OK; }
+    if (what == ZK_TUNE_DEDUPE_TABLE) { c->dedupe_table = value < 0 ? 0 : (value > 2 ? 0 : value); return ZK_OK; }
     if (what == ZK_TUNE_KWAY) { c->kway = value < 0 ? 0 : (value > 2 ? 2 : value); return ZK_OK; }
     if (what == ZK_TUNE_TILE_SORT) { c->tile_sort = value ? 1 : 0; return ZK_OK; }
     if (what == ZK_TUNE_TAG_PASS) { c->tag_pass = value ? 1 : 0; return ZK_OK; }
diff --git a/zotmer_amd/csrc/dedupe.hpp b/zotmer_amd/csrc/dedupe.hpp
--- a/zotmer_amd/csrc/dedupe.hpp
+++ b/zotmer_amd/csrc/dedupe.hpp
@@ -40,6 +40,6 @@
 #define DD_PHASE(k) do { } while (0)
 #endif
 
-int launch_dedupe2(zk_ctx* c, const DedupeArgs& a, bool tagin, int variant, bool unsorted);
+int launch_dedupe2(zk_ctx* c, const DedupeArgs& a, bool tagin, int variant, bool unsorted, bool small_table = false);
 
 }
diff --git a/zotmer_amd/csrc/dedupe2.hip b/zotmer_amd/csrc/dedupe2.hip
--- a/zotmer_amd/csrc/dedupe2.hip
+++ b/zotmer_amd/csrc/dedupe2.hip
@@ -3,9 +3,10 @@
 
 namespace zk {
 
-template <int BLOCK_, int BATCH_, int ITEMS_>
+constexpr int D2_ALL = 11264, D2_ALL_SMALL = 6656;
+template <int BLOCK_, int BATCH_, int ITEMS_, int ALL_ = D2_ALL>
 struct Dedupe2Smem {
-    static constexpr int BLOCK = BLOCK_, BATCH = BATCH_, ITEMS = ITEMS_, TILE = BLOCK * ITEMS, NW = BLOCK / 64, ALL = 11264, SPT = ALL / BLOCK,
+    static constexpr int BLOCK = BLOCK_, BATCH = BATCH_, ITEMS = ITEMS_, TILE = BLOCK * ITEMS, NW = BLOCK / 64, ALL = ALL_, SPT = ALL / BLOCK,
                          NB = 1024, SIDE = 64 + 64 * BATCH;
     static_assert(ALL % BLOCK == 0 && ALL % 8 == 0 && ITEMS % BATCH == 0 && ITEMS % 4 == 0, "whole rounds, whole quads, whole batches");
     alignas(16) u32 keys[ALL];
@@ -17,8 +18,8 @@
     u32 ticket;
     u32 nout;
 };
-template <int BLOCK_, int BATCH_, int ITEMS_>
-struct Dedupe2MirrorSmem : Dedupe2Smem<BLOCK_, BATCH_, ITEMS_> {
+template <int BLOCK_, int BATCH_, int ITEMS_, int ALL_ = D2_ALL>
+struct Dedupe2MirrorSmem : Dedupe2Smem<BLOCK_, BATCH_, ITEMS_, ALL_> {
     u32 bins[2][MIRROR_RADIX];
     u64 mbase;
 };
@@ -326,11 +327,11 @@
     DD_PHASE(5);
 }
 
-template <int BLOCK, int BATCH, int ITEMS, bool TAGIN, bool UNSORTED, bool MIRROR = false>
-__global__ __launch_bounds__(BLOCK, 2 * BLOCK / 256) void dedupe2_kernel(DedupeArgs a) {
-    using S = typename std::conditional<MIRROR, Dedupe2MirrorSmem<BLOCK, BATCH, ITEMS>, Dedupe2Smem<BLOCK, BATCH, ITEMS>>::type;
+template <int BLOCK, int BATCH, int ITEMS, bool TAGIN, bool UNSORTED, bool MIRROR = false, int ALL = D2_ALL, int WGS = 2>
+__global__ __launch_bounds__(BLOCK, WGS * BLOCK / 256) void dedupe2_kernel(DedupeArgs a) {
+    using S = typename std::conditional<MIRROR, Dedupe2MirrorSmem<BLOCK, BATCH, ITEMS, ALL>, Dedupe2Smem<BLOCK, BATCH, ITEMS, ALL>>::type;
     __shared__ S sm;
-    static_assert(sizeof(S) <= 80 * 1024, "two workgroups per CU");
+    static_assert((sizeof(S) + 1279) / 1280 * 1280 * WGS <= 160 * 1024, "WGS workgroups per CU");
     Dedupe2Next<ITEMS> st;
     if constexpr (MIRROR)
         for (int q = threadIdx.x; q < 2 * MIRROR_RADIX; q += BLOCK) (&sm.bins[0][0])[q] = 0;
@@ -368,13 +369,15 @@
     }
 }
 
-int launch_dedupe2(zk_ctx* c, const DedupeArgs& a, bool tagin, int variant, bool unsorted) {
-    const u32 want = 2u * (u32)c->num_cus;
+int launch_dedupe2(zk_ctx* c, const DedupeArgs& a, bool tagin, int variant, bool unsorted, bool small_table) {
+    const u32 want = ((small_table && a.m_out) ? 3u : 2u) * (u32)c->num_cus;
     const u32 grid = a.chunks < want ? a.chunks : want;
     if (a.m_out) {
         if (!tagin || !unsorted || !a.m_cursor || !a.m_hist || a.m_passes < 1 || a.m_passes > 2 || a.m_bits[0] > MIRROR_RBITS || a.m_bits[1] > MIRROR_RBITS)
             return fail(c, ZK_EINTERNAL, "launch_dedupe2: mirror words with %d passes, tags %d, unsorted %d", a.m_passes, (int)tagin, (int)unsorted);
-        if ((variant & 3) == 1) hipLaunchKernelGGL((dedupe2_kernel<512, 1, 8, true, true, true>), dim3(grid), dim3(512), 0, c->stream, a);
+        if (small_table && (variant & 3) == 1) hipLaunchKernelGGL((dedupe2_kernel<512, 1, 8, true, true, true, D2_ALL_SMALL, 3>), dim3(grid), dim3(512), 0, c->stream, a);
+        else if (small_table) hipLaunchKernelGGL((dedupe2_kernel<512, 2, 8, true, true, true, D2_ALL_SMALL, 3>), dim3(grid), dim3(512), 0, c->stream, a);
+        else if ((variant & 3) == 1) hipLaunchKernelGGL((dedupe2_kernel<512, 1, 8, true, true, true>), dim3(grid), dim3(512), 0, c->stream, a);
         else hipLaunchKernelGGL((dedupe2_kernel<512, 2, 8, true, true, true>), dim3(grid), dim3(512), 0, c->stream, a);
         ZK_HIP(c, hipGetLastError());
         return ZK_OK;
diff --git a/zotmer_amd/csrc/dedupe_blocks.hip b/zotmer_amd/csrc/dedupe_blocks.hip
--- a/zotmer_amd/csrc/dedupe_blocks.hip
+++ b/zotmer_amd/csrc/dedupe_blocks.hip
@@ -408,13 +408,13 @@
     else hipLaunchKernelGGL((dedupe_kernel<false, false>), dim3(grid), dim3(1024), 0, c->stream, d);
 }
 
-static int dedupe_launch(zk_ctx* c, DedupeArgs& a, bool two_per_cu, bool unsorted, DedupeResult* r) {
+static int dedupe_launch(zk_ctx* c, DedupeArgs& a, bool two_per_cu, bool unsorted, bool small_table, DedupeResult* r) {
     prof_begin(c, ZK_PROF_RLE, (a.tin ? 4 : 8) * a.n);
     if (two_per_cu) {
         ZK_TRY(arena_alloc(c, sizeof(u32) * a.chunks, (void**)&a.retry));
         a.n_retry = (u32*)&c->d_scalars->dedupe_n_retry;
         a.limit = (u32)c->dedupe_limit;
-        ZK_TRY(launch_dedupe2(c, a, a.tin != nullptr, c->dedupe_variant, unsorted));
+        ZK_TRY(launch_dedupe2(c, a, a.tin != nullptr, c->dedupe_variant, unsorted, small_table));
     } else launch_one_per_cu(c, a);
     prof_end(c);
     ZK_HIP(c, hipGetLastError());
@@ -472,7 +472,8 @@
     DedupeArgs a = {};
     const bool two_per_cu = key_bits - b <= 32 && c->dedupe_variant >= 0;
     ZK_TRY(dedupe_lists(c, keys, n, key_bits, b, pack, work, max_chunks, tags, tag_cuts, unsorted, two_per_cu, mirror, a, r));
-    ZK_TRY(dedupe_launch(c, a, two_per_cu, r->unsorted, r));
+    const bool small_table = a.m_out && (c->dedupe_table == 1 || (c->dedupe_table == 0 && mirror->per_block && mirror->per_block <= 6656 / 2));
+    ZK_TRY(dedupe_launch(c, a, two_per_cu, r->unsorted, small_table, r));
     r->flags = (uint32_t)c->h_scalars->dedupe_flags;
     r->n_big = (uint32_t)c->h_scalars->dedupe_n_big;
     if (r->n_big > DEDUPE_BIG_CAP) r->flags |= 1;
diff --git a/zotmer_amd/csrc/encode_tile.hpp b/zotmer_amd/csrc/encode_tile.hpp
--- a/zotmer_amd/csrc/encode_tile.hpp
+++ b/zotmer_amd/csrc/encode_tile.hpp
@@ -1,7 +1,16 @@
 #pragma once
+#include "../../include/zotk.h"
 #include "common.hpp"
 
 namespace zk {
+
+__host__ __device__ __forceinline__ bool middle_flips(int K, u64 x) { return (x >> K) & 1ull; }
+__host__ __device__ __forceinline__ u64 strand_key(int mode, int K, u64 x, u64 xb) {
+    if (mode == ZK_KEYS_CANONICAL) return x < xb ? x : xb;
+    if (mode == ZK_KEYS_MIDDLE) return middle_flips(K, x) ? xb : x;
+    return x;
+}
+__host__ __device__ __forceinline__ bool one_key_mode(int mode) { return mode == ZK_KEYS_CANONICAL || mode == ZK_KEYS_MIDDLE; }
 
 template <int T> struct TileImage {
     static constexpr int NCH = T / 16 + 3;
diff --git a/zotmer_amd/csrc/internal.hpp b/zotmer_amd/csrc/internal.hpp
--- a/zotmer_amd/csrc/internal.hpp
+++ b/zotmer_amd/csrc/internal.hpp
@@ -92,6 +92,7 @@
     int stream_pass = 1;
     int tag_words = 2;
     int dedupe_variant = 0;
+    int dedupe_table = 0;
     int dedupe_limit = 65536;
     int tag_pass = 0;
     int kway = 1;
@@ -218,7 +219,7 @@
 constexpr int MIRROR_RBITS = 9, MIRROR_RADIX = 1 << MIRROR_RBITS;
 struct MirrorHist { int passes; int shift[4]; int bits[4]; u64* raw; };
 int sort_keys_upper_counted(zk_ctx* c, u64* keys, u64* alt, uint64_t n, int key_bits, int lo_bit, u64* counted, u64** result);
-struct DedupeMirror { u64* out = nullptr; uint64_t cap = 0; int K = 0; };
+struct DedupeMirror { u64* out = nullptr; uint64_t cap = 0; int K = 0; uint64_t per_block = 0; };
 struct DedupeResult {
     uint64_t n_out = 0;
     uint32_t flags = 0;
diff --git a/zotmer_amd/csrc/pipeline.hip b/zotmer_amd/csrc/pipeline.hip
--- a/zotmer_amd/csrc/pipeline.hip
+++ b/zotmer_amd/csrc/pipeline.hip
@@ -268,6 +268,7 @@
     bool blocks_mirror;
     bool blocks_strands;
     bool blocks_unsorted;
+    bool middle;
     CountRoute low_route() const { return fused_bit ? COUNT_FUSED : collapse_bit ? COUNT_RUNS : COUNT_SORTED; }
 };
 
@@ -299,6 +300,7 @@
     p.blocks_mirror = !canonical_only && p.pack && p.dedupe_bit == MIRROR_GROUP_BITS && mirror_groups(K);
     p.blocks_strands = p.blocks_mirror && (K & 1) && c->strand_blocks;
     p.blocks_unsorted = p.blocks_mirror && (K & 1) && (c->strand_blocks == 1 || c->strand_blocks >= 3);
+    p.middle = (K & 1) && !both && !canonical_only && p.dedupe_bit && p.tags && p.blocks_strands && p.blocks_unsorted && !c->tag_pass;
     return p;
 }
 
@@ -315,13 +317,14 @@
     uint64_t n = 0;
     StreamTags tags;
     bool presampled = false;
+    uint64_t per_block = 0;
     CountRoute route = COUNT_SORTED;
 };
 
 static int sort_by_plan(zk_ctx* c, const KmerizePlan& p, const u8* stream, uint64_t n_bytes, const SortBufs& b, bool may_replan,
                         uint64_t acgt[4], Sorted* s) {
     const int K = p.K;
-    StreamSrc src{stream, n_bytes, K, p.both ? ZK_KEYS_BOTH : ZK_KEYS_CANONICAL, 0};
+    StreamSrc src{stream, n_bytes, K, p.both ? ZK_KEYS_BOTH : p.middle ? ZK_KEYS_MIDDLE : ZK_KEYS_CANONICAL, 0};
     s->route = p.dedupe_bit ? COUNT_BLOCKS : p.low_route();
     bool sorted = false;
     if (p.dedupe_bit) {
@@ -331,10 +334,12 @@
         const int rc = sort_stream(c, src, b.a, b.b, b.cap_keys, &s->n, acgt, &s->keys);
         if (rc < 0) return rc;
         src.sample = nullptr; src.tags = nullptr;
+        if (rc == 1) src.mode = ZK_KEYS_CANONICAL;
         if (rc == 1 && may_replan && p.replan_pays) { s->route = COUNT_REPLAN; return ZK_OK; }
         if (rc == 1) s->route = p.tile_top ? COUNT_TILES : p.low_route();
         else sorted = true;
         s->presampled = smp.seen >= 4096;
+        s->per_block = smp.distinct / 4;
     } else if (p.look) {
         StreamSample smp = prefix_sample(K, p.look_bits);
         smp.want_distinct = true;
@@ -422,6 +427,7 @@
     if (!s.presampled) ZK_TRY(dedupe_pass(c, s.keys, s.n, 2 * K, p.dedupe_bit, pk, s.other, b.cap_keys, &d, &n_in, (1u << 20) / per + 4, tg, s.tags.cuts));
     if (s.presampled || (!(d.flags & 1) && (double)d.n_out <= REPEAT_RATIO * (double)n_in)) {
         DedupeMirror mo;
+        if (p.middle) mo.per_block = s.presampled ? s.per_block : d.n_out / (d.chunks ? d.chunks : 1) + 1;
         const uint64_t tag_words = align256(4 * s.n) / 8;
         if (tg && p.blocks_strands && p.blocks_unsorted && c->strand_blocks != 4 && tag_words < b.cap_keys) {
             mo.out = s.keys + tag_words; mo.cap = b.cap_keys - tag_words; mo.K = K;
diff --git a/zotmer_amd/csrc/radix_sort.hip b/zotmer_amd/csrc/radix_sort.hip
--- a/zotmer_amd/csrc/radix_sort.hip
+++ b/zotmer_amd/csrc/radix_sort.hip
@@ -115,7 +115,7 @@
 #pragma unroll
             for (int i = 0; i < ITEMS; i++) {
                 const u64 x = xs[i & 15], xb = xr[i & 15];
-                key[i] = (a.mode == ZK_KEYS_CANONICAL) ? (x < xb ? x : xb) : x;
+                key[i] = strand_key(a.mode, K, x, xb);
                 if (COUNT && ((ok16 >> i) & 1u)) acgt += (1u << (8 * (u32)(x & 3))) + (1u << (8 * (u32)(xb & 3)));
             }
             live = ok16;
@@ -126,7 +126,7 @@
                 u64 x;
                 const bool ok = window_at(*img, p, K, x);
                 const u64 xb = revcomp(K, x);
-                key[i] = (a.mode == ZK_KEYS_CANONICAL) ? (x < xb ? x : xb) : x;
+                key[i] = strand_key(a.mode, K, x, xb);
                 live |= (ok ? 1u : 0u) << i;
                 if (COUNT && ok) acgt += (1u << (8 * (u32)(x & 3))) + (1u << (8 * (u32)(xb & 3)));
             }
@@ -264,7 +264,7 @@
                     u64 x, xb;
                     if (wg.get(i, x, xb)) {
                         pk += (1u << (8 * (u32)(x & 3))) + (1u << (8 * (u32)(xb & 3)));
-                        const u64 kk = (h.src.mode == ZK_KEYS_CANONICAL) ? (x < xb ? x : xb) : x;
+                        const u64 kk = strand_key(h.src.mode, h.src.K, x, xb);
                         if (h.plan.passes == 2) {
                             atomicAdd(&bins[(u32)(kk >> h.plan.shift[0]) & ((1u << h.plan.bits[0]) - 1u)], 1u);
                             atomicAdd(&bins[C::RADIX + ((u32)(kk >> h.plan.shift[1]) & ((1u << h.plan.bits[1]) - 1u))], 1u);
@@ -815,7 +815,7 @@
 #pragma unroll
                 for (int i = 0; i < ITEMS; i++) {
                     const u64 x = xs[i & 15], xb = xr[i & 15];
-                    key[i] = (a.mode == ZK_KEYS_CANONICAL) ? (x < xb ? x : xb) : x;
+                    key[i] = strand_key(a.mode, a.K, x, xb);
                 }
                 __syncthreads();
             }
@@ -1094,12 +1094,12 @@
     StreamPlan s;
     s.top = (src.hi_bit > 0 && src.hi_bit < 2 * src.K) ? src.hi_bit : 2 * src.K;
     s.plan = make_plan(s.top - src.lo_bit, rbits, src.lo_bit);
-    s.sampling = src.sample && cap >= 4ull * SAMPLE_CAP && src.mode == ZK_KEYS_CANONICAL;
+    s.sampling = src.sample && cap >= 4ull * SAMPLE_CAP && one_key_mode(src.mode);
     s.ranged = c->stream_pass != 0;
     const uint64_t n_pad = ((n + 63) & ~63ull) + 64;
     s.planes = s.ranged && c->tag_pass && src.tags && s.plan.passes == 2 && s.plan.shift[0] == 32 && s.plan.bits[0] == 9 && s.plan.bits[1] == 9 &&
                src.mode == ZK_KEYS_CANONICAL && 2 * src.K > 32 && n >= 4096 && 4 * n_pad + 2 * n + 64 <= 8 * cap;
-    s.tags = src.tags && pipe && s.plan.passes == 2 && s.plan.shift[0] <= 32 && src.mode == ZK_KEYS_CANONICAL;
+    s.tags = src.tags && pipe && s.plan.passes == 2 && s.plan.shift[0] <= 32 && one_key_mode(src.mode);
     s.straddle = c->tag_words >= 2 && pipe;
     return s;
 }
diff --git a/zotmer_amd/csrc/stream_pass.hip b/zotmer_amd/csrc/stream_pass.hip
--- a/zotmer_amd/csrc/stream_pass.hip
+++ b/zotmer_amd/csrc/stream_pass.hip
@@ -157,13 +157,15 @@
     const int np = h.plan.passes;
     const u64 mask = ~0ull >> (64 - 2 * K);
     const u32 mlo = (u32)mask, mhi = (u32)(mask >> 32);
-    const bool canon = CANON_T == 1 ? true : h.mode == ZK_KEYS_CANONICAL;
-    const bool both = CANON_T != 1 && h.mode == ZK_KEYS_BOTH;
+    const int kmode = CANON_T == 1 ? ZK_KEYS_CANONICAL : CANON_T == 2 ? ZK_KEYS_MIDDLE : h.mode;
+    const bool canon = kmode == ZK_KEYS_CANONICAL;
+    const bool both = CANON_T < 0 && h.mode == ZK_KEYS_BOTH;
     const u32 sh0 = (u32)h.plan.shift[0] - (HI ? 32u : 0u), sh1 = (u32)h.plan.shift[1] - (HI ? 32u : 0u);
     const u32 dm0 = (1u << h.plan.bits[0]) - 1u, dm1 = (1u << h.plan.bits[1]) - 1u;
     const u32 base1 = h.binbase[1];
     const u32 nb0 = (u32)h.plan.bits[0], nb1 = (u32)h.plan.bits[1];
     const u32 ssh = (u32)h.sample_shift - (HI ? 32u : 0u);
+    const u32 sbits = (u32)(2 * K - h.sample_shift);
     const typename std::conditional<HI, u32, u64>::type sval = (typename std::conditional<HI, u32, u64>::type)h.sample_value;
     u32 a0 = 0, a1 = 0, a2 = 0, a3 = 0, nl_count = 0, bad_count = 0;
     u32 rec = 0, m = 0, step_m = 0;
@@ -229,6 +231,7 @@
         const u32 V16 = mine ? (u32)(v >> 48) : 0u;
         WindowWords<SH_NW> ww;
         ww.init(a, b, 0u, K);
+        const int midb = (int)((a << (K - 1)) >> 32);
         if (h.acgt) {
             const u32 Vs = spread16(V16);
             const u32 ff = (u32)(a >> 32);
@@ -245,11 +248,16 @@
             const u32 inc = (V16 >> (15 - i)) & 1u;
             typename std::conditional<HI, u32, u64>::type kd;
             if constexpr (HI) {
-                const u32 xh = ww.xhi(i) & mhi, bh = ww.bhi(i) & mhi;
-                kd = canon ? (xh < bh ? xh : bh) : xh;
+                if constexpr (CANON_T == 2) {
+                    const u32 flip = (u32)__builtin_amdgcn_sbfe(midb, 31 - 2 * i, 1);
+                    kd = (ww.bhi(i) & flip) | (ww.xhi(i) & ~flip);
+                } else {
+                    const u32 xh = ww.xhi(i) & mhi, bh = ww.bhi(i) & mhi;
+                    kd = canon ? (xh < bh ? xh : bh) : xh;
+                }
             } else {
                 const u64 x = ((u64)(ww.xhi(i) & mhi) << 32) | (ww.xlo(i) & mlo), xb = ((u64)(ww.bhi(i) & mhi) << 32) | (ww.blo(i) & mlo);
-                kd = canon ? (x < xb ? x : xb) : x;
+                kd = strand_key(kmode, K, x, xb);
             }
             if constexpr (TWO && HI) {
 #ifdef ZK_PHASES
@@ -274,7 +282,8 @@
                 }
             }
             if constexpr (HI) {
-                if (h.sample) hits |= ((kd >> ssh) == sval ? 1u : 0u) << (15 - i);
+                if constexpr (CANON_T == 2) { if (h.sample) hits |= (__builtin_amdgcn_ubfe(kd, ssh, sbits) == sval ? 1u : 0u) << (15 - i); }
+                else if (h.sample) hits |= ((kd >> ssh) == sval ? 1u : 0u) << (15 - i);
             } else if (h.sample && inc && (kd >> ssh) == sval) {
                 const u32 at = atomicAdd(h.sample_n, 1u);
                 if (at < h.sample_cap) h.sample[at] = kd;
@@ -286,7 +295,7 @@
             for (int i = 0; i < SH_NW; i++) {
                 if ((hits >> (15 - i)) & 1u) {
                     const u64 x = (((u64)ww.xhi(i) << 32) | ww.xlo(i)) & mask, xb = (((u64)ww.bhi(i) << 32) | ww.blo(i)) & mask;
-                    const u64 kk = canon ? (x < xb ? x : xb) : x;
+                    const u64 kk = CANON_T == 2 ? (middle_flips(K, x) ? xb : x) : canon ? (x < xb ? x : xb) : x;
                     const u32 at = atomicAdd(h.sample_n, 1u);
                     if (at < h.sample_cap) h.sample[at] = kk;
                 }
@@ -392,8 +401,9 @@
     u32 anybad;
 };
 
-template <int RBITS, int G, bool CANON, bool FAST, bool PLANES = false>
+template <int RBITS, int G, bool CANON, bool FAST, bool PLANES = false, bool MID = false>
 __global__ __launch_bounds__(P0_BLOCK, 4) void stream_pass0_kernel(P0Args a) {
+    static_assert(CANON || !MID, "the middle-base rule is a rule for one key per window");
     using S = P0Smem<RBITS, G>;
     constexpr int RADIX = S::RADIX, NW = P0_NW, BLOCK = P0_BLOCK;
     static_assert(S::CAP < (1 << 14) && G <= 16 && RBITS <= 14, "unit_pack");
@@ -587,7 +597,7 @@
                 const u64 x = ((u64)(ww.xhi(i) & mhi) << 32) | (FAST ? ww.xlo(i) : (ww.xlo(i) & mlo));
                 if constexpr (CANON) {
                     const u64 xb = ((u64)(ww.bhi(i) & mhi) << 32) | (FAST ? ww.blo(i) : (ww.blo(i) & mlo));
-                    key[i] = x < xb ? x : xb;
+                    key[i] = MID ? (middle_flips(K, x) ? xb : x) : (x < xb ? x : xb);
                 } else {
                     const u64 xb = ((u64)(ww.bhi(i) & mhi) << 32) | (FAST ? ww.blo(i) : (ww.blo(i) & mlo));
                     key[i] = rev ? xb : x;
@@ -712,8 +722,9 @@
     u32 anybad;
 };
 
-template <int RBITS, bool CANON, bool FAST>
+template <int RBITS, bool CANON, bool FAST, bool MID = false>
 __global__ __launch_bounds__(PW_BLOCK) void stream_pass0_wide_kernel(P0Args a) {
+    static_assert(CANON || !MID, "the middle-base rule is a rule for one key per window");
     constexpr int G = 16;
     using S = P0WideSmem<RBITS, G>;
     constexpr int RADIX = S::RADIX, NW = PW_NW, BLOCK = PW_BLOCK;
@@ -834,7 +845,7 @@
             for (int i = 0; i < NW; i++) {
                 const u64 x = ((u64)(ww.xhi(i) & mhi) << 32) | (FAST ? ww.xlo(i) : (ww.xlo(i) & mlo));
                 const u64 xb = ((u64)(ww.bhi(i) & mhi) << 32) | (FAST ? ww.blo(i) : (ww.blo(i) & mlo));
-                if constexpr (CANON) key[i] = x < xb ? x : xb;
+                if constexpr (CANON) key[i] = MID ? (middle_flips(K, x) ? xb : x) : (x < xb ? x : xb);
                 else key[i] = rev ? xb : x;
             }
         }
@@ -1000,9 +1011,11 @@
     ZK_HIP(c, hipMemsetAsync(ghist, 0, sizeof(u64) * MAX_PASSES * gstride, c->stream));
     if (d_acgt) ZK_HIP(c, hipMemsetAsync(d_acgt, 0, sizeof(u64) * 4, c->stream));
     const u32 grid = h.ranges * h.split;
+    const bool two = plan.passes == 2 && !both;
+    if (hi && !two && mode == ZK_KEYS_MIDDLE) return fail(c, ZK_EINTERNAL, "stream_hist: the middle-base rule with %d passes", plan.passes);
     prof_begin(c, ZK_PROF_HIST_STREAM, n_bytes);
-    const bool two = plan.passes == 2 && !both;
     if (hi && two && mode == ZK_KEYS_CANONICAL) hipLaunchKernelGGL((stream_hist_kernel<true, true, 1>), dim3(grid), dim3(SH_BLOCK), nb * sizeof(u32), c->stream, h);
+    else if (hi && two && mode == ZK_KEYS_MIDDLE) hipLaunchKernelGGL((stream_hist_kernel<true, true, 2>), dim3(grid), dim3(SH_BLOCK), nb * sizeof(u32), c->stream, h);
     else if (hi && two) hipLaunchKernelGGL((stream_hist_kernel<true, true>), dim3(grid), dim3(SH_BLOCK), nb * sizeof(u32), c->stream, h);
     else if (hi) hipLaunchKernelGGL((stream_hist_kernel<true, false>), dim3(grid), dim3(SH_BLOCK), nb * sizeof(u32), c->stream, h);
     else if (two) hipLaunchKernelGGL((stream_hist_kernel<false, true>), dim3(grid), dim3(SH_BLOCK), nb * sizeof(u32), c->stream, h);
@@ -1026,9 +1039,10 @@
     a.ranges = rows.ranges;
     a.by_record = (uniform && a.tl.rec) ? 1 : 0;
     a.shift = shift; a.bits = bits; a.offs = rows.offs; a.rows = rows.rows; a.kout = kout; a.n = n; a.err = c->d_err; a.dbg = c->dbg; a.dbg_mode = variant >> 8; a.split_stores = (variant & 0xff) == 3;
-    const bool canon = mode == ZK_KEYS_CANONICAL, fast = 2 * K > 32 && shift >= 32;
+    const bool canon = one_key_mode(mode), mid = mode == ZK_KEYS_MIDDLE, fast = 2 * K > 32 && shift >= 32;
+    if (mid && !(K & 1)) return fail(c, ZK_EINTERNAL, "stream_pass0: the middle-base rule at even K = %d", K);
     if (planes) {
-        if (!canon || !fast || rows.wide) return fail(c, ZK_EINTERNAL, "stream_pass0: planes need the canonical fast plan and the 512-thread kernel");
+        if (!canon || mid || !fast || rows.wide) return fail(c, ZK_EINTERNAL, "stream_pass0: planes need the canonical fast plan and the 512-thread kernel");
         a.dig_out = planes->dig; a.dig_shift = planes->shift; a.dig_mask = (1u << planes->bits) - 1u;
         prof_begin(c, ZK_PROF_PASS_STREAM, n_bytes + 6 * n);
         hipLaunchKernelGGL((stream_pass0_kernel<9, 8, true, true, true>), dim3(rows.ranges), dim3(P0_BLOCK), 0, c->stream, a);
@@ -1038,11 +1052,15 @@
     }
     prof_begin(c, ZK_PROF_PASS_STREAM, n_bytes + 8 * n);
     if (rows.wide) {
-        if (canon && fast) hipLaunchKernelGGL((stream_pass0_wide_kernel<9, true, true>), dim3(grid), dim3(PW_BLOCK), 0, c->stream, a);
+        if (mid && fast) hipLaunchKernelGGL((stream_pass0_wide_kernel<9, true, true, true>), dim3(grid), dim3(PW_BLOCK), 0, c->stream, a);
+        else if (mid) hipLaunchKernelGGL((stream_pass0_wide_kernel<9, true, false, true>), dim3(grid), dim3(PW_BLOCK), 0, c->stream, a);
+        else if (canon && fast) hipLaunchKernelGGL((stream_pass0_wide_kernel<9, true, true>), dim3(grid), dim3(PW_BLOCK), 0, c->stream, a);
         else if (canon) hipLaunchKernelGGL((stream_pass0_wide_kernel<9, true, false>), dim3(grid), dim3(PW_BLOCK), 0, c->stream, a);
         else if (fast) hipLaunchKernelGGL((stream_pass0_wide_kernel<9, false, true>), dim3(grid), dim3(PW_BLOCK), 0, c->stream, a);
         else hipLaunchKernelGGL((stream_pass0_wide_kernel<9, false, false>), dim3(grid), dim3(PW_BLOCK), 0, c->stream, a);
-    } else if (canon && fast) hipLaunchKernelGGL((stream_pass0_kernel<9, 8, true, true>), dim3(grid), dim3(P0_BLOCK), 0, c->stream, a);
+    } else if (mid && fast) hipLaunchKernelGGL((stream_pass0_kernel<9, 8, true, true, false, true>), dim3(grid), dim3(P0_BLOCK), 0, c->stream, a);
+    else if (mid) hipLaunchKernelGGL((stream_pass0_kernel<9, 8, true, false, false, true>), dim3(grid), dim3(P0_BLOCK), 0, c->stream, a);
+    else if (canon && fast) hipLaunchKernelGGL((stream_pass0_kernel<9, 8, true, true>), dim3(grid), dim3(P0_BLOCK), 0, c->stream, a);
     else if (canon) hipLaunchKernelGGL((stream_pass0_kernel<9, 8, true, false>), dim3(grid), dim3(P0_BLOCK), 0, c->stream, a);
     else if (fast) hipLaunchKernelGGL((stream_pass0_kernel<9, 8, false, true>), dim3(grid), dim3(P0_BLOCK), 0, c->stream, a);
     else hipLaunchKernelGGL((stream_pass0_kernel<9, 8, false, false>), dim3(grid), dim3(P0_BLOCK), 0, c->stream, a);
diff --git a/zotmer_amd/native.py b/zotmer_amd/native.py
--- a/zotmer_amd/native.py
+++ b/zotmer_amd/native.py
@@ -428,7 +428,7 @@
 
     TUNE_IDS = dict(sort_variant=1, pairs_variant=2, short_sort=3, side_div=4, xcd_group=5, comm_chunk=6, early_collapse=7,
                     packed_pairs=8, wide_tiles=9, stream_pass=10, stream_ranges=11, tag_words=12, dedupe_variant=13, dedupe_limit=14,
-                    dedupe_bits=15, comm_self_loop=16, tag_pass=17, kway=18, tile_sort=19, strand_blocks=20)
+                    dedupe_bits=15, comm_self_loop=16, tag_pass=17, kway=18, tile_sort=19, strand_blocks=20, dedupe_table=21)
 
     def tune(self, **knobs):
         for name in knobs:
```

Result: faster. 168.2, median of 6 (+1.0%).
